# Damorgal/Biprojection-Multimodal-Transformer

Hardware: AMD Instinct MI355X
Metric: training samples/sec (fwd+bwd) BPMulT hidden=768, 3-modal unaligned, at 1/2/4/8 MI355X (higher is better)
Workload: dtype bf16; 1 GPU; BPMulT hidden=768 3-modal unaligned: IEMOCAP-shape synthetic mmtrvat d=768 H=12 layers=8 L/V/A=20/500/400->512; per_gpu_batch=8, global_batch=8, parallelism=dp1, world=1, dropout=README rates (attn .1/0/0, relu .1, res .1, embed .25)

## Files before the change

biprojection-multimodal-transformer_amd/_lib.py:

```python
from __future__ import annotations

import ctypes as C
import os
import subprocess

import torch

_HERE = os.path.dirname(os.path.abspath(__file__))
CSRC = os.path.join(_HERE, "csrc")
LIB_PATH = os.environ.get("BPMULT_LIB", os.path.join(_HERE, "libbpmult_hip.so"))
SOURCES = ("gemm.hip", "attention.hip", "attn_maps.hip", "attn_dbias.hip", "rows_pack.hip", "rows_norm.hip", "rows_elem.hip", "adam.hip", "bert_embed.hip", "loss.hip", "eval.hip", "tail.hip", "frontend.hip", "prof.hip")
HEADERS = ("bpm_common.h", "bpm_launch.h", "bpm_prof.h", "gemm_dma.h", "rows_common.h", "attn_common.h")
ARCH = "gfx950"
PROF_KINDS = {"gemm_nt": 0, "gemm_nn": 1, "gemm_tn": 2, "attn_fwd": 3, "attn_bwd_dq": 4, "attn_bwd_dkv": 5,
              "gemm_dma_nt": 13, "gemm_dma_nn": 14, "gemm_dma_tn": 15, "attn_maps": 16, "attn_bwd_dbias": 17}

ABI_VERSION = 5
LAB_LIB_PATH = os.path.join(_HERE, "..", "build", "lab", "libbpmult_hip_lab.so")
BPM_F32, BPM_BF16, BPM_BF16X3 = 0, 1, 2
GEMM_NT, GEMM_NN, GEMM_TN = 0, 1, 2
OUT_F32, OUT_CT, OUT_HEADS = 0, 1, 2
F_ACCUM, F_RELU, F_ATOMIC, F_KPAD, F_BACKGROUND = 1, 2, 4, 8, 16
F_A_OVERLAP, F_B_OVERLAP = 32, 64
F_CT_NARROW, F_BATCHED = 128, 256
# ... 26 lines not shown
    if not force and fresh():
        return out
    os.makedirs(objdir, exist_ok=True)
    os.makedirs(os.path.dirname(os.path.abspath(out)), exist_ok=True)
    hipcc = os.environ.get("HIPCC", "/opt/rocm/bin/hipcc")
    common = [hipcc, f"--offload-arch={ARCH}", "-O3", "-std=c++17", "-fPIC"] + list(flags)

    def compile_one(src):
        obj = os.path.join(objdir, os.path.basename(src)[:-4] + ".o")
        if not force and os.path.exists(obj) and os.path.getmtime(obj) >= max(os.path.getmtime(src), newest_hdr):
            return obj
        tmp = f"{obj}.{os.getpid()}.tmp"
        cmd = common + ["-c", src, "-o", tmp]
        if verbose:
            print(" ".join(cmd))
        subprocess.run(cmd, check=True)
        os.replace(tmp, obj)
        return obj

    with open(os.path.join(objdir, ".lock"), "w") as lock:
        fcntl.flock(lock, fcntl.LOCK_EX)
        try:
            if not force and fresh():
                return out
            with ThreadPoolExecutor(max_workers=min(4, os.cpu_count() or 1)) as ex:
                objs = list(ex.map(compile_one, srcs))
            tmp = f"{out}.{os.getpid()}.tmp"
            cmd = [hipcc, f"--offload-arch={ARCH}", "-shared", "-fPIC", "-o", tmp] + objs
            if verbose:
                print(" ".join(cmd))
            subprocess.run(cmd, check=True)
            os.replace(tmp, out)
        finally:
            fcntl.flock(lock, fcntl.LOCK_UN)
    return out


def build_lab(force: bool = False) -> str:
    return build(force=force, out=LAB_LIB_PATH, flags=("-DBPM_LAB",))


class GemmProblem(C.Structure):
    _fields_ = [("A", C.c_void_p), ("B", C.c_void_p), ("C", C.c_void_p),
                ("M", C.c_int), ("N", C.c_int), ("K", C.c_int),
                ("lda", C.c_int), ("ldb", C.c_int), ("ldc", C.c_int),
                ("bias_n", C.c_void_p), ("bias_m", C.c_void_p),
                ("resid", C.c_void_p), ("ldr", C.c_int),
                ("gate", C.c_void_p), ("ldg", C.c_int), ("gate_scale", C.c_float),
                ("alpha", C.c_float), ("drop_p", C.c_float), ("drop_site", C.c_uint32),
                ("colsum", C.c_void_p),
                ("flags", C.c_int), ("out_kind", C.c_int), ("splitk", C.c_int),
                ("heads_B", C.c_int), ("heads_H", C.c_int), ("heads_T", C.c_int),
                ("heads_dh", C.c_int), ("heads_dhp", C.c_int), ("colsum_a", C.c_void_p),
                ("batch", C.c_int), ("batch_stride_a", C.c_int), ("batch_stride_b", C.c_int), ("batch_stride_c", C.c_int)]


class AttnProblem(C.Structure):
    _fields_ = [("Q", C.c_void_p), ("K", C.c_void_p), ("V", C.c_void_p),
                ("O", C.c_void_p), ("ldo", C.c_int), ("lse", C.c_void_p),
                ("dO", C.c_void_p), ("delta", C.c_void_p),
                ("dQ", C.c_void_p), ("lddq", C.c_int),
                ("dK", C.c_void_p), ("lddk", C.c_int),
                ("dV", C.c_void_p), ("lddv", C.c_int),
                ("B", C.c_int), ("H", C.c_int), ("T", C.c_int), ("S", C.c_int),
                ("dh", C.c_int), ("dhp", C.c_int), ("mask_off", C.c_int),
                ("dq_scale", C.c_float), ("drop_p", C.c_float), ("drop_site", C.c_uint32),
                ("q_pos0", C.c_int), ("q_stride", C.c_int),
                ("dS", C.c_void_p), ("Pd", C.c_void_p), ("xs_b", C.c_int), ("xs_h", C.c_int), ("xs_q", C.c_int)]


class AttnKMask(C.Structure):
    _fields_ = [("mask", C.c_void_p), ("ldm", C.c_int)]


class AttnAMask(C.Structure):
    _fields_ = [("mask", C.c_void_p), ("ldm", C.c_int), ("maskT", C.c_void_p), ("ldt", C.c_int)]


class AttnHMask(C.Structure):
    _fields_ = [("mask", C.c_void_p), ("ldm", C.c_int), ("maskT", C.c_void_p), ("ldt", C.c_int),
                ("head_stride", C.c_int64), ("head_strideT", C.c_int64)]


class AttnDBias(C.Structure):
    _fields_ = [("dB", C.c_void_p), ("lddb", C.c_int), ("head_stride", C.c_int64)]


class GeluProblem(C.Structure):
    _fields_ = [("u", C.c_void_p), ("ldu", C.c_int), ("u_is_ct", C.c_int), ("g", C.c_void_p), ("ldg", C.c_int),
                ("dg", C.c_void_p), ("lddg", C.c_int), ("du", C.c_void_p), ("lddu", C.c_int), ("R", C.c_int), ("C", C.c_int)]


class BertEmbedProblem(C.Structure):
    _fields_ = [("ids", C.c_void_p), ("seg", C.c_void_p), ("word", C.c_void_p), ("pos", C.c_void_p), ("type", C.c_void_p),
                ("V", C.c_int), ("P", C.c_int), ("Tt", C.c_int), ("gamma", C.c_void_p), ("beta", C.c_void_p),
                ("B", C.c_int), ("L", C.c_int), ("x", C.c_void_p), ("xc", C.c_void_p), ("ldc", C.c_int),
                ("s", C.c_void_p), ("mean", C.c_void_p), ("rstd", C.c_void_p), ("bad", C.c_void_p),
                ("drop_p", C.c_float), ("drop_site", C.c_uint32)]


class BertScatterProblem(C.Structure):
    _fields_ = [("ds", C.c_void_p), ("sorted_ids", C.c_void_p), ("perm", C.c_void_p), ("seg", C.c_void_p),
                ("dword", C.c_void_p), ("dpos", C.c_void_p), ("dtype", C.c_void_p),
                ("V", C.c_int), ("Tt", C.c_int), ("B", C.c_int), ("L", C.c_int), ("padding_idx", C.c_int64),
                ("ws", C.c_void_p), ("ws_bytes", C.c_size_t)]


# ... 34 lines not shown
    _fields_ = [("off4", C.c_size_t), ("n4", C.c_uint), ("blk0", C.c_uint), ("dst", C.c_void_p),
                ("rows", C.c_int), ("cols", C.c_int), ("dst_ld", C.c_int), ("group", C.c_int)]


class AdamGroup(C.Structure):
    _fields_ = [("lr", C.c_float), ("beta1", C.c_float), ("beta2", C.c_float), ("eps", C.c_float), ("weight_decay", C.c_float),
                ("decoupled", C.c_int), ("step", C.c_int), ("pad_", C.c_int)]


class AdamSet(C.Structure):
    _fields_ = [("param", C.c_void_p), ("grad", C.c_void_p), ("exp_avg", C.c_void_p), ("exp_avg_sq", C.c_void_p), ("n", C.c_size_t)]


def adam_set_group(set_index: int, group: int) -> int:
    w = (set_index << ADAM_SET_SHIFT) | (group & 0xff)
    return w - (1 << 32) if w >= 1 << 31 else w


class SumsqSeg(C.Structure):
    _fields_ = [("p", C.c_void_p), ("n", C.c_size_t), ("blk0", C.c_uint), ("pad_", C.c_uint)]


class LossDesc(C.Structure):
    _fields_ = [("kind", C.c_int), ("reduction", C.c_int), ("B", C.c_int), ("C", C.c_int),
                ("logits", C.c_void_p), ("ld", C.c_int), ("target", C.c_void_p), ("ldt", C.c_int), ("weight", C.c_void_p),
                ("ignore_index", C.c_int64), ("loss", C.c_void_p), ("dlogits_unit", C.c_void_p), ("ldd", C.c_int),
                ("bad", C.c_void_p), ("ws", C.c_void_p), ("ws_bytes", C.c_size_t)]


class EvalDesc(C.Structure):
    _fields_ = [("kind", C.c_int), ("C", C.c_int), ("capacity", C.c_int), ("max_batches", C.c_int),
                ("score", C.c_void_p), ("predict", C.c_void_p), ("raw", C.c_void_p), ("target", C.c_void_p),
                ("pred", C.c_void_p), ("label", C.c_void_p), ("losses", C.c_void_p), ("bad", C.c_void_p),
                ("logits", C.c_void_p), ("ld", C.c_int), ("targets", C.c_void_p), ("ldt", C.c_int), ("loss", C.c_void_p),
                ("B", C.c_int), ("n0", C.c_int), ("batch_index", C.c_int),
                ("N", C.c_int), ("nbatches", C.c_int), ("result", C.c_void_p), ("counts", C.c_void_p),
                ("ws", C.c_void_p), ("ws_bytes", C.c_size_t)]


class SplitProblem(C.Structure):
    _fields_ = [("src", C.c_void_p), ("dst", C.c_void_p), ("R", C.c_int), ("C", C.c_int), ("ld", C.c_int), ("ldp", C.c_int)]


class EmbedProblem(C.Structure):
    _fields_ = [("x", C.c_void_p), ("out", C.c_void_p), ("T", C.c_int), ("B", C.c_int), ("accumulate", C.c_int),
                ("drop_p", C.c_float), ("drop_site", C.c_uint32), ("pos0", C.c_int), ("pos_stride", C.c_int)]


class KvSourceProblem(C.Structure):
    _fields_ = [("xk", C.c_void_p), ("xv", C.c_void_p), ("T", C.c_int), ("B", C.c_int), ("pos0", C.c_int), ("pos_stride", C.c_int),
                ("drop_p_k", C.c_float), ("drop_site_k", C.c_uint32), ("drop_p_v", C.c_float), ("drop_site_v", C.c_uint32),
                ("khat", C.c_void_p), ("vhat", C.c_void_p), ("ld", C.c_int),
                ("mean_k", C.c_void_p), ("rstd_k", C.c_void_p), ("mean_v", C.c_void_p), ("rstd_v", C.c_void_p),
                ("gk", C.c_void_p), ("gv", C.c_void_p), ("dxk", C.c_void_p), ("dxv", C.c_void_p)]


class LnProblem(C.Structure):
    _fields_ = [("x", C.c_void_p), ("gamma", C.c_void_p), ("beta", C.c_void_p),
                ("out", C.c_void_p), ("ldo", C.c_int), ("out_f32", C.c_int),
                ("mean", C.c_void_p), ("rstd", C.c_void_p), ("R", C.c_int),
                ("dy", C.c_void_p), ("ldy", C.c_int), ("add", C.c_void_p), ("dx", C.c_void_p),
                ("dgamma", C.c_void_p), ("dbeta", C.c_void_p),
                ("cast", C.c_void_p), ("ldc", C.c_int), ("cast_colsum", C.c_void_p),
                ("drop_p", C.c_float), ("drop_site", C.c_uint32)]


class CastProblem(C.Structure):
    _fields_ = [("a", C.c_void_p), ("lda", C.c_int), ("a_is_ct", C.c_int),
                ("b", C.c_void_p), ("ldb", C.c_int),
                ("dst_ct", C.c_void_p), ("ldd", C.c_int), ("ct_cols", C.c_int),
                ("dst_f32", C.c_void_p), ("ldf", C.c_int),
                ("colsum", C.c_void_p), ("R", C.c_int), ("C", C.c_int),
                ("drop_p", C.c_float), ("drop_site", C.c_uint32)]


class GmuProblem(C.Structure):
    _fields_ = [("a1", C.c_void_p), ("a2", C.c_void_p), ("ag", C.c_void_p), ("x1", C.c_void_p), ("x2", C.c_void_p),
                ("out", C.c_void_p), ("dout", C.c_void_p), ("da1", C.c_void_p), ("da2", C.c_void_p), ("dag", C.c_void_p),
                ("ldg", C.c_int), ("dx1", C.c_void_p), ("dx2", C.c_void_p), ("R", C.c_int)]


class AddnProblem(C.Structure):
    _fields_ = [("out", C.c_void_p), ("src", C.c_void_p * 8), ("n_in", C.c_int), ("count", C.c_size_t)]


class ExpandProblem(C.Structure):
    _fields_ = [("q", C.c_void_p), ("dO", C.c_void_p), ("qexp", C.c_void_p), ("dOexp", C.c_void_p), ("Pd", C.c_void_p),
                ("dbias", C.c_void_p), ("B", C.c_int), ("H", C.c_int), ("T", C.c_int), ("S", C.c_int), ("dh", C.c_int),
                ("dhp", C.c_int), ("ld", C.c_int)]


class TailDesc(C.Structure):
    _fields_ = [("B", C.c_int), ("d", C.c_int), ("n", C.c_int), ("C", C.c_int), ("N", C.c_int * 3),
                ("top", C.c_void_p * 3), ("mid", C.c_void_p * 3), ("extra", C.c_void_p),
                ("Wh", C.c_void_p * 4), ("Wg", C.c_void_p * 4),
                ("W1", C.c_void_p), ("b1", C.c_void_p), ("W2", C.c_void_p), ("b2", C.c_void_p), ("Wo", C.c_void_p), ("bo", C.c_void_p),
                ("out_dropout", C.c_float), ("drop_site", C.c_uint32),
                ("x", C.c_void_p), ("z", C.c_void_p), ("t", C.c_void_p), ("h", C.c_void_p), ("p1", C.c_void_p), ("y", C.c_void_p),
                ("logits", C.c_void_p)]


class TailGrads(C.Structure):
    _fields_ = [("dlogits", C.c_void_p), ("dz", C.c_void_p), ("dWh", C.c_void_p * 4), ("dWg", C.c_void_p * 4),
                ("dW1", C.c_void_p), ("db1", C.c_void_p), ("dW2", C.c_void_p), ("db2", C.c_void_p), ("dWo", C.c_void_p), ("dbo", C.c_void_p),
                ("dtop", C.c_void_p * 3), ("dmid", C.c_void_p * 3), ("dextra", C.c_void_p),
                ("dy", C.c_void_p), ("dp1", C.c_void_p), ("dh", C.c_void_p), ("dzp", C.c_void_p), ("dtp", C.c_void_p), ("dx", C.c_void_p)]

# ... 64 lines not shown
    "bpm_grad_sumsq_blocks": [_P, C.c_size_t],
    "bpm_grad_sumsq_ws_bytes": [C.c_uint],
    "bpm_grad_sumsq": [_P, _I, C.c_uint, _F, _F, _P, _P, C.c_size_t, _P, _P],
    "bpm_loss_ws_bytes": [_I, _I, _I, _I],
    "bpm_loss_fwd": [C.POINTER(LossDesc), _P],
    "bpm_loss_bwd": [C.POINTER(LossDesc), _P, _I, _P, _I, _P],
    "bpm_eval_ws_bytes": [_I, _I, _I],
    "bpm_eval_update": [C.POINTER(EvalDesc), _P],
    "bpm_eval_finalize": [C.POINTER(EvalDesc), _P],
    "bpm_eval_image_bytes": [_I, _I, _I, _I],
    "bpm_eval_pack": [C.POINTER(EvalDesc), _I, _I, _I, _I, _P, C.c_size_t, _P],
    "bpm_eval_merge": [C.POINTER(EvalDesc), _P, C.c_size_t, _I, C.POINTER(_I), C.POINTER(_I), _P],
    "bpm_stream_create": [_I, C.POINTER(C.c_void_p)],
    "bpm_stream_priority_range": [C.POINTER(_I), C.POINTER(_I)],
    "bpm_prof_enable": [C.c_uint],
    "bpm_prof_collect": [_I, C.POINTER(C.c_double), C.POINTER(C.c_double), C.POINTER(_I)],
    "bpm_prof_collect2": [_I, C.POINTER(C.c_double), C.POINTER(C.c_double), C.POINTER(C.c_double), C.POINTER(_I)],
}

_lib = None


class HipLibraryError(RuntimeError):
    pass


def load(path: str) -> C.CDLL:
    if not os.path.exists(path):
        raise HipLibraryError(
            f"{path} not found: run `python -c 'import __graft_entry__ as g; g.build()'` "
            "(hipcc --offload-arch=gfx950). The BPMulT hot path has no CPU/PyTorch fallback.")
    L = C.CDLL(path)
    for name, args in SIGNATURES.items():
        fn = getattr(L, name)
        fn.argtypes = args
        fn.restype = C.c_char_p if name == "bpm_error_string" else C.c_size_t if name.endswith("_bytes") else C.c_int
    v = L.bpm_version()
    if v != ABI_VERSION:
        raise HipLibraryError(f"{path}: ABI version {v}, this package binds version {ABI_VERSION} (include/bpmult_hip.h): rebuild it")
    return L


def lib() -> C.CDLL:
    global _lib
    if _lib is None:
        _lib = load(LIB_PATH)
    return _lib


def bind_lab(L: C.CDLL) -> C.CDLL:
    L.bpm_debug_gemm_force.argtypes = [C.c_int]
    L.bpm_debug_attn_pair.argtypes = [C.c_int]
    L.bpm_debug_gemm_choice.argtypes = [C.c_int, C.c_int, C.POINTER(GemmProblem), C.c_int, C.c_int, C.POINTER(C.c_int)]
    L.bpm_debug_rows_dry.argtypes = [C.c_int]
    L.bpm_debug_rows_last.argtypes = [C.c_int, C.c_char_p, C.c_int, C.POINTER(C.c_uint), C.POINTER(C.c_uint), C.POINTER(C.c_void_p)]
    return L


class lab_library:

    def __enter__(self) -> C.CDLL:
        global _lib
        self._prev = _lib
        _lib = bind_lab(load(LAB_LIB_PATH))
        return _lib

    def __exit__(self, *exc) -> None:
        global _lib
        try:
            _lib.bpm_debug_gemm_force(-1)
            _lib.bpm_debug_attn_pair(7)
        finally:
            _lib = self._prev


_prof_mask = 0


def prof_enable(mask: int) -> None:
    global _prof_mask
    lib().bpm_prof_enable(mask)
    _prof_mask = mask


def prof_enabled() -> bool:
    return _prof_mask != 0


_DEBUG_SYNC = bool(int(os.environ.get("BPMULT_DEBUG_SYNC", "0")))


def check(rc: int, what: str) -> None:
    if rc != 0:
        msg = lib().bpm_error_string(rc)
        raise RuntimeError(f"{what} failed (code {rc}): {msg.decode() if msg else '?'}")
    if _DEBUG_SYNC:
        import sys
        import torch
        print(f"[bpmult] {what} ...", end="", file=sys.stderr, flush=True)
        torch.cuda.synchronize()
        print(" ok", file=sys.stderr, flush=True)
```

biprojection-multimodal-transformer_amd/csrc/gemm.hip:

```cpp
#include <cstdlib>
#include <type_traits>

#include "bpm_common.h"
#include "bpm_prof.h"
#include "../../include/bpmult_hip.h"

namespace {

constexpr int BM = 128, BN = 64, WM = 2, WN = 2;
constexpr int NTHREADS = 64 * WM * WN;
constexpr int TM = BM / WM / 16;
constexpr int TN = BN / WN / 16;
constexpr int BPM_TILED_MINW = 5;
constexpr int BPM_SETPRIO = 0;
constexpr int BPM_DEEP_TN = 2;
constexpr int BPM_DEEP_FWD = 1;
constexpr int KS_FWD = 1, KS_WGRAD = 2;
struct Prob {
    const char* X; const char* Y; char* C;
    int M, N, K;
    int ldx, ldy, ldc;
    const float* bias_n; const float* bias_m;
    const float* resid; const char* gate;
    int ldr, ldg; float gate_scale;
    float alpha;
    float* colsum;
    float* colsum_x;
    DropCfg drop;
    int flags;
    int out_kind;
    int hB, hH, hT, hdh, hdhp;
    int tile0, tiles_m, tiles_n, splitk;
};
static_assert(sizeof(Prob) == 168, "Prob layout");

struct Group {
    const uint64_t* seedp;
    int nprob;
    int total_tiles;
    Prob p[BPM_GEMM_MAX_GROUP];
};
static_assert(sizeof(Group) + 16 <= 4096, "the problem table travels as a kernel argument (4 KB)");

BPM_DEV int swz4(int row) { return (-(row >> 2)) & 3; }

template <typename CT>
BPM_DEV void store_ct4(char* C, size_t off_elems, const float (&v)[4], int nvalid) {
    CT* p = (CT*)C + off_elems;
    if (nvalid == 4 && ((off_elems & 3) == 0)) {
        if constexpr (sizeof(CT) == 4) {
            *(f32x4*)p = f32x4{v[0], v[1], v[2], v[3]};
        } else {
            bf16x4 o;
#pragma unroll
            for (int r = 0; r < 4; ++r) o[r] = (bf16_t)v[r];
            *(bf16x4*)p = o;
        }
    } else {
#pragma unroll
        for (int r = 0; r < 4; ++r)
            if (r < nvalid) p[r] = Tr<CT>::from_f(v[r]);
    }
}

template <typename CT>
BPM_DEV void epilogue_tile(const Prob& P, const DropCfg& drop, bool lead, int m, int nb, const f32x4& acc, float (&csum)[4]) {
    if (m >= P.M) return;
    const bool atomic = (P.flags & BPM_GEMM_ATOMIC) != 0;
    const bool accum = (P.flags & BPM_GEMM_ACCUM) != 0;
    const bool relu = (P.flags & BPM_GEMM_RELU) != 0;
    const bool full = nb + 3 < P.N;
    float v[4];
    float bn[4] = {0.f, 0.f, 0.f, 0.f}, rs[4] = {0.f, 0.f, 0.f, 0.f}, gt[4] = {1.f, 1.f, 1.f, 1.f};
    if (lead && P.bias_n) {
        const float* bp = P.bias_n + nb;
        if (full && (((uintptr_t)bp & 15) == 0)) { const f32x4 t = *(const f32x4*)bp; bn[0] = t[0]; bn[1] = t[1]; bn[2] = t[2]; bn[3] = t[3]; }
        else {
#pragma unroll
            for (int q = 0; q < 4; ++q) if (nb + q < P.N) bn[q] = bp[q];
        }
    }
    if (lead && P.resid) {
        const float* rp = P.resid + (size_t)m * P.ldr + nb;
        if (full && (((uintptr_t)rp & 15) == 0)) { const f32x4 t = *(const f32x4*)rp; rs[0] = t[0]; rs[1] = t[1]; rs[2] = t[2]; rs[3] = t[3]; }
// ... 305 lines not shown
        if (KCONTIG) {
            if (SWZ) {
                const int r = lane & 15, g = lane >> 4;
                return *(const typename Tr<CT>::frag*)(img + (r0 + r) * 64 + ((g ^ swz4(r0 + r)) << 4));
            }
            return read_rowfrag<CT>(img, ROW_STRIDE, r0, ks, lane);
        }
        return Tr<CT>::read_tr(img, STRIDE, ks * Tr<CT>::KSTEP, r0, lane, Tr<CT>::TR_CTILE);
    }
};

BPM_DEV const Prob& pick_problem(const Group& grp, int& bid) {
    int pi = 0;
#pragma unroll 1
    for (int i = 1; i < grp.nprob; ++i)
        if (bid >= grp.p[i].tile0) pi = i;
    bid -= grp.p[pi].tile0;
    return grp.p[pi];
}

#ifdef BPM_GEMM_TRACE
__device__ unsigned long long g_trace[8192 * 16];
#define BPM_TRACE(slot) do { if (threadIdx.x == 0 && blockIdx.x < 8192 && (slot) < 16) \
        g_trace[blockIdx.x * 16 + (slot)] = __builtin_amdgcn_s_memrealtime(); } while (0)
#else
#define BPM_TRACE(slot) do { } while (0)
#endif

template <typename CT, bool XK, bool YK, int KSTEPS, bool DEEP = false, bool FAST = false, int BMT = BM>
__global__ __launch_bounds__(NTHREADS) __attribute__((amdgpu_waves_per_eu((!XK && !YK) ? (BMT == 64 ? 6 : 4) : BPM_TILED_MINW, (!XK && !YK) ? (BMT == 64 ? 6 : 4) : BPM_TILED_MINW))) void gemm_tiled_kernel(const Group grp) {
    typedef Side<CT, XK, BMT, KSTEPS, XK && !YK> SX;
    constexpr int TMT = BMT / WM / 16;
    typedef Side<CT, YK, BN, KSTEPS, false> SY;
    constexpr int STAGE = SX::IMG_BYTES + SY::IMG_BYTES;
    __shared__ __attribute__((aligned(16))) char smem[2 * STAGE];

    const int tid = threadIdx.x, lane = tid & 63, wave = tid >> 6;
    const int wm = wave / WN, wn = wave % WN;

    BPM_TRACE(0);
    int bid = xcd_remap(blockIdx.x, gridDim.x);
    const Prob& P = pick_problem(grp, bid);
    if (BPM_BASE_PRIO && XK && !(P.flags & BPM_GEMM_BACKGROUND)) __builtin_amdgcn_s_setprio(BPM_BASE_PRIO);
    const int tiles = P.tiles_m * P.tiles_n;
    const int split = bid / tiles;
    const int t = bid % tiles;
    const int m0 = (t / P.tiles_n) * BMT, n0 = (t % P.tiles_n) * BN;
    const bool batched = (P.flags & BPM_GEMM_BATCHED) != 0;

    constexpr int BK = SX::BK;
    const int nkt_all = (P.K + BK - 1) / BK;
    const int per = batched ? nkt_all : (nkt_all + P.splitk - 1) / P.splitk;
    const int kt_lo = batched ? 0 : split * per;
    const int kt_hi = min(nkt_all, kt_lo + per);

    f32x4 acc[TN][TMT];
#pragma unroll
    for (int a = 0; a < TN; ++a)
#pragma unroll
        for (int b = 0; b < TMT; ++b) acc[a][b] = f32x4{0.f, 0.f, 0.f, 0.f};

    constexpr int XBT = (TMT + WN - 1) / WN;
    [[maybe_unused]] f32x4 xs[XBT];
    [[maybe_unused]] bool do_xs = false;
    if constexpr (!XK && !YK) {
        do_xs = P.colsum_x != nullptr && n0 == 0;
#pragma unroll
        for (int b = 0; b < XBT; ++b) xs[b] = f32x4{0.f, 0.f, 0.f, 0.f};
    }
    auto compute = [&](const char* ix) {
        const char* iy = ix + SX::IMG_BYTES;
#pragma unroll
        for (int ks = 0; ks < KSTEPS; ++ks) {
            typename Tr<CT>::frag fx[TMT], fy[TN];
#pragma unroll
            for (int b = 0; b < TMT; ++b) fx[b] = SX::frag(ix, wm * (BMT / WM) + 16 * b, ks, lane);
            if constexpr (!XK && !YK) {
                if (do_xs) {
                    typename Tr<CT>::frag one;
#pragma unroll
                    for (int j = 0; j < Tr<CT>::EPC; ++j) one[j] = Tr<CT>::from_f(1.0f);
#pragma unroll
                    for (int b = 0; b < TMT; ++b)
                        if (b / XBT == wn) xs[b % XBT] = Tr<CT>::mma(one, fx[b], xs[b % XBT]);
                }
            }
#pragma unroll
            for (int a = 0; a < TN; ++a) fy[a] = SY::frag(iy, wn * (BN / WN) + 16 * a, ks, lane);
            if (BPM_SETPRIO) __builtin_amdgcn_s_setprio(1);
#pragma unroll
            for (int a = 0; a < TN; ++a)
#pragma unroll
                for (int b = 0; b < TMT; ++b) acc[a][b] = Tr<CT>::mma(fy[a], fx[b], acc[a][b]);
            if (BPM_SETPRIO) __builtin_amdgcn_s_setprio(0);
        }
    };

    const char* const Xp = P.X + (batched ? (size_t)split * (size_t)P.hB * sizeof(CT) : (size_t)0);
    const char* const Yp = P.Y + (batched ? (size_t)split * (size_t)P.hH * sizeof(CT) : (size_t)0);
    const int ldx = P.ldx, ldy = P.ldy, Mb = P.M, Nb = P.N, Kb = P.K;
    [[maybe_unused]] __amdgpu_buffer_rsrc_t rsx, rsy;
    [[maybe_unused]] int vx[SX::PER_THREAD], vy[SY::PER_THREAD];
    [[maybe_unused]] int stepx = 0, stepy = 0;
    if constexpr (FAST) {
        constexpr int E = Tr<CT>::EPC;
        const int kceil = (Kb + BK - 1) / BK * BK;
        const int wx = XK ? kceil : (Mb + E - 1) / E * E, wy = YK ? kceil : (Nb + E - 1) / E * E;
        rsx = __builtin_amdgcn_make_buffer_rsrc((void*)Xp, 0, ((XK ? Mb : Kb) - 1) * ldx * (int)sizeof(CT) + ((P.flags & BPM_GEMM_A_OVERLAP) ? wx : min(wx, ldx)) * (int)sizeof(CT), 0x00020000);
        rsy = __builtin_amdgcn_make_buffer_rsrc((void*)Yp, 0, ((YK ? Nb : Kb) - 1) * ldy * (int)sizeof(CT) + ((P.flags & BPM_GEMM_B_OVERLAP) ? wy : min(wy, ldy)) * (int)sizeof(CT), 0x00020000);
        SX::voffsets(ldx, m0, tid, vx);
        SY::voffsets(ldy, n0, tid, vy);
        stepx = SX::stage_step(ldx);
        stepy = SY::stage_step(ldy);
    }
    auto LD = [&](int kt, u32x4 (&rx_)[SX::PER_THREAD], u32x4 (&ry_)[SY::PER_THREAD], uint32_t& mx_, uint32_t& my_) {
        if constexpr (FAST) {
            SX::load_fast(rsx, vx, kt * stepx, rx_);
            SY::load_fast(rsy, vy, kt * stepy, ry_);
            mx_ = 0xFFFFFFFFu; my_ = 0xFFFFFFFFu;
        } else {
            mx_ = SX::load(Xp, ldx, m0, Mb, kt * BK, Kb, rx_, tid);
            my_ = SY::load(Yp, ldy, n0, Nb, kt * BK, Kb, ry_, tid);
        }
    };
    if constexpr (DEEP) {
        u32x4 rx0[SX::PER_THREAD], ry0[SY::PER_THREAD], rx1[SX::PER_THREAD], ry1[SY::PER_THREAD];
        uint32_t mx0 = 0, my0 = 0, mx1 = 0, my1 = 0;
        auto ld0 = [&](int kt) { LD(kt, rx0, ry0, mx0, my0); };
        auto ld1 = [&](int kt) { LD(kt, rx1, ry1, mx1, my1); };
        auto st0 = [&](char* img) { SX::store(img, rx0, mx0, tid); SY::store(img + SX::IMG_BYTES, ry0, my0, tid); };
        auto st1 = [&](char* img) { SX::store(img, rx1, mx1, tid); SY::store(img + SX::IMG_BYTES, ry1, my1, tid); };
        ld0(kt_lo);
        st0(smem);
        ld1(kt_lo + 1);
        __syncthreads();
        BPM_TRACE(1);
        int cur = 0;
#pragma unroll 1
        for (int kt = kt_lo; kt < kt_hi; kt += 2) {
            ld0(kt + 2);
            compute(smem + cur * STAGE);
            if (kt + 1 < kt_hi) st1(smem + (cur ^ 1) * STAGE);
            __syncthreads();
            BPM_TRACE(2 + kt - kt_lo);
            cur ^= 1;
            if (kt + 1 >= kt_hi) break;
            ld1(kt + 3);
            compute(smem + cur * STAGE);
            if (kt + 2 < kt_hi) st0(smem + (cur ^ 1) * STAGE);
            __syncthreads();
            BPM_TRACE(3 + kt - kt_lo);
            cur ^= 1;
        }
    } else {
        u32x4 rx[SX::PER_THREAD], ry[SY::PER_THREAD];
        uint32_t mx = 0, my = 0;
        LD(kt_lo, rx, ry, mx, my);
        SX::store(smem, rx, mx, tid);
        SY::store(smem + SX::IMG_BYTES, ry, my, tid);
        __syncthreads();
        BPM_TRACE(1);
        int cur = 0;
#pragma unroll 1
        for (int kt = kt_lo; kt < kt_hi; ++kt) {
            const bool more = kt + 1 < kt_hi;
            LD(kt + 1, rx, ry, mx, my);
            compute(smem + cur * STAGE);
            if (more) {
                char* nx = smem + (cur ^ 1) * STAGE;
                SX::store(nx, rx, mx, tid);
                SY::store(nx + SX::IMG_BYTES, ry, my, tid);
            }
            __syncthreads();
            BPM_TRACE(2 + kt - kt_lo);
            cur ^= 1;
        }
    }

// ... 164 lines not shown
    int force_dma;
    int two_mask;
    bool narrow_dma;
};
#ifdef BPM_LAB
int env_int(const char* name, int unset) { const char* v = std::getenv(name); return v ? std::atoi(v) : unset; }
Lab g_lab = {-1, env_int("BPMULT_TWO_MASK", 7), env_int("BPMULT_NARROW_DMA", 1) != 0};
#else
constexpr Lab g_lab = {-1, 7, true};
#endif

int num_cus() {
    static int ncu = 0;
    if (!ncu) {
        int dev = 0;
        hipDeviceProp_t prop;
        ncu = (hipGetDevice(&dev) == hipSuccess && hipGetDeviceProperties(&prop, dev) == hipSuccess && prop.multiProcessorCount > 0)
                  ? prop.multiProcessorCount : 256;
    }
    return ncu;
}

bool bounded_ok(const bpm_gemm_problem& q, int variant, int sz) {
    const bool xk = variant != BPM_GEMM_TN, yk = variant == BPM_GEMM_NT;
    const int stage_b = 64 * (variant == BPM_GEMM_NT ? KS_FWD : 1);
    const bool aov = (q.flags & BPM_GEMM_A_OVERLAP) != 0, bov = (q.flags & BPM_GEMM_B_OVERLAP) != 0;
    bool ok = (q.flags & BPM_GEMM_KPAD_ZERO) != 0;
    if (xk) ok = ok && (aov ? q.K % 64 == 0 : ((long)q.lda * sz) % stage_b == 0 && (long)q.K <= q.lda);
    if (yk) ok = ok && (bov ? q.K % 64 == 0 : ((long)q.ldb * sz) % stage_b == 0 && (long)q.K <= q.ldb);
    const long bx = ((long)(xk ? q.M : q.K) - 1) * q.lda * sz + (long)(aov ? (xk ? q.K : q.M) : q.lda) * sz;
    const long by = ((long)(yk ? q.N : q.K) - 1) * q.ldb * sz + (long)(bov ? (yk ? q.K : q.N) : q.ldb) * sz;
    return ok && bx < (1l << 31) - 65536 && by < (1l << 31) - 65536;
}

int check_group(int dtype, int variant, const bpm_gemm_problem* probs, int nprob) {
    if (nprob < 1 || nprob > BPM_GEMM_MAX_GROUP || !probs) return BPM_ERR_ARG;
    if (variant != BPM_GEMM_NT && variant != BPM_GEMM_NN && variant != BPM_GEMM_TN) return BPM_ERR_ARG;
    if (dtype != BPM_F32 && dtype != BPM_BF16 && dtype != BPM_BF16X3) return BPM_ERR_ARG;
    const int sz = dtype == BPM_F32 ? 4 : 2;
    bool fast = true, overlap = false;
    for (int i = 0; i < nprob && fast; ++i) {
        overlap = overlap || (probs[i].flags & (BPM_GEMM_A_OVERLAP | BPM_GEMM_B_OVERLAP)) != 0;
        fast = bounded_ok(probs[i], variant, sz);
    }
    if (overlap && !fast) return BPM_ERR_ARG;
    for (int i = 0; i < nprob; ++i) {
        const bpm_gemm_problem& q = probs[i];
        if (q.M < 1 || q.N < 1 || q.K < 1 || !q.A || !q.B || !q.C) return BPM_ERR_ARG;
        if ((q.lda * sz) % 16 || (q.ldb * sz) % 16) return BPM_ERR_ALIGN;
        if (((uintptr_t)q.A | (uintptr_t)q.B) & 15) return BPM_ERR_ALIGN;
        if (q.colsum_a && (variant != BPM_GEMM_TN || q.splitk > 1)) return BPM_ERR_ARG;
        if (q.out_kind == BPM_OUT_HEADS && (q.heads_B < 1 || q.heads_dh < 1 || q.heads_H * q.heads_dh != q.N)) return BPM_ERR_ARG;
        if (q.splitk > 1 && !((q.flags & BPM_GEMM_ATOMIC) && q.out_kind == BPM_OUT_F32)) return BPM_ERR_ARG;
        if (q.flags & BPM_GEMM_BATCHED) {
            const uintptr_t al = (uintptr_t)q.C | (uintptr_t)q.bias_n;
            if (dtype == BPM_BF16X3 || q.batch < 1 || q.batch > 4096 || q.splitk > 1 || q.out_kind == BPM_OUT_HEADS || q.bias_m || q.resid ||
                q.gate || q.colsum || q.colsum_a || q.drop_p != 0.f || (q.flags & (BPM_GEMM_ATOMIC | BPM_GEMM_ACCUM)) ||
                (q.N & 3) || (q.ldc & 3) || (al & 15) || q.batch_stride_a < 0 || q.batch_stride_b < 0 || q.batch_stride_c < 0 ||
                ((q.batch_stride_a * sz) & 15) || ((q.batch_stride_b * sz) & 15) || (q.batch_stride_c & 3))
                return BPM_ERR_ARG;
        }
    }
    return 0;
}

struct GroupShape {
    bool fast = true;
    bool legal = true;
    bool big = true;
    bool narrow = true;
    bool skinny = true;
    bool xs_any = false;
    long kmin = 1l << 30, kmax = 0, nmax = 0, mmax = 0;
    long t128 = 0;
    long wg128 = 0;
    long t256 = 0, t320 = 0, tiles_narrow = 0;
};

GroupShape summarise(int dtype, int variant, const bpm_gemm_problem* probs, int nprob) {
    const bool x3 = dtype == BPM_BF16X3, xk = variant != BPM_GEMM_TN, yk = variant == BPM_GEMM_NT;
    const int sz = dtype == BPM_F32 ? 4 : 2;
    GroupShape s;
    for (int i = 0; i < nprob; ++i) {
        const bpm_gemm_problem& q = probs[i];
        s.fast = s.fast && bounded_ok(q, variant, sz);
        const long kceil = ((long)q.K + DK - 1) / DK * DK;
        bool legal = q.splitk <= 1 && !(q.flags & (BPM_GEMM_ATOMIC | BPM_GEMM_BATCHED)) && (!xk || (q.flags & BPM_GEMM_A_OVERLAP) || kceil <= q.lda) &&
                     (!yk || (q.flags & BPM_GEMM_B_OVERLAP) || kceil <= q.ldb);
        if (x3) {
            const long pa = q.lda / 2, pb = q.ldb / 2, m128 = ((long)q.M + 127) / 128 * 128, n128 = ((long)q.N + 127) / 128 * 128;
            legal = legal && !(q.flags & (BPM_GEMM_A_OVERLAP | BPM_GEMM_B_OVERLAP)) && (q.lda & 1) == 0 && (q.ldb & 1) == 0 &&
                    (xk ? kceil <= pa : m128 <= pa) && (yk ? kceil <= pb : n128 <= pb) && (pa * 2) % 16 == 0 && (pb * 2) % 16 == 0;
        }
        const uintptr_t al = (uintptr_t)q.bias_n | (uintptr_t)q.resid | (uintptr_t)q.C | (uintptr_t)q.gate;
        s.legal = s.legal && legal && (q.N & 3) == 0 && (al & 15) == 0 && ((q.ldr | q.ldc | q.ldg) & 3) == 0 && !q.bias_m &&
                  !(q.resid && (q.flags & BPM_GEMM_ACCUM));
        const long tm = (q.M + 255) / 256, tn = (q.N + 255) / 256, tn_narrow = (q.N + 127) / 128;
        s.big = s.big && q.M >= 256 && q.N >= 256 && q.K >= 256 && (double)q.M * q.N >= 0.8 * (double)(tm * 256) * (double)(tn * 256);
        s.narrow = s.narrow && q.M >= 256 && q.N >= 128 && q.K >= 256 && (double)q.M * q.N >= 0.75 * (double)(tm * 256) * (double)(tn_narrow * 128);
        s.skinny = s.skinny && q.M <= 16 && q.splitk <= 1 &&
                   !(q.flags & (BPM_GEMM_ATOMIC | BPM_GEMM_A_OVERLAP | BPM_GEMM_B_OVERLAP | BPM_GEMM_BATCHED)) &&
                   ((long)q.lda * sz) % 64 == 0 && (variant != BPM_GEMM_NT || ((long)q.ldb * sz) % 64 == 0);
        s.xs_any = s.xs_any || q.colsum_a != nullptr;
        s.kmin = q.K < s.kmin ? q.K : s.kmin;
        s.kmax = q.K > s.kmax ? q.K : s.kmax;
        s.nmax = q.N > s.nmax ? q.N : s.nmax;
        s.mmax = q.M > s.mmax ? q.M : s.mmax;
        const long t = (long)((q.M + BM - 1) / BM) * ((q.N + BN - 1) / BN);
        s.t128 += t * (q.splitk > 1 ? q.splitk : 1);
        s.wg128 += t * ((q.flags & BPM_GEMM_BATCHED) ? q.batch : q.splitk > 1 ? q.splitk : 1);
        s.t256 += tm * tn;
        s.t320 += (q.M + 319) / 320 * tn;
        s.tiles_narrow += tm * tn_narrow;
    }
    return s;
}

Choice choose(const GroupShape& s, int dtype, int variant, int nprob, int ncu, const Lab& lab) {
    const bool x3 = dtype == BPM_BF16X3, tn = variant == BPM_GEMM_TN;
    int dma = -1;
    if ((dtype == BPM_BF16 || x3) && s.fast && s.legal && (lab.force_dma != -2 || x3)) {
        const bool big = x3 || (s.big && !(tn && s.t256 * 8 < (long)ncu * 5));
        if (lab.force_dma >= 0 && !x3) dma = lab.force_dma == K_DMA_TALL && tn ? -1 : lab.force_dma;
        else if (big) {
            dma = tn ? K_DMA_2 : K_DMA_3;
            if (!tn) {
                const long r256 = (s.t256 + ncu - 1) / ncu, r320 = (s.t320 + ncu - 1) / ncu;
                if (r320 * 320 * 21 < r256 * 256 * 20) dma = K_DMA_TALL;
            }
            const bool nt = variant == BPM_GEMM_NT;
            const bool two_tn = (lab.two_mask & 1) && tn && !s.xs_any && s.kmin >= 1024 && s.mmax <= 1024;
            const bool kv = (lab.two_mask & 2) && nt && nprob >= 12 && s.nmax <= 1024;
            const bool fc1 = (lab.two_mask & 4) && nt && s.nmax >= 2048 && s.kmax <= 1024;
            if (!x3 && (two_tn || kv || fc1)) dma = K_DMA_TWO;
        }
        else if (lab.narrow_dma && !tn && s.narrow && s.tiles_narrow >= ncu) dma = K_DMA_TWO;
    }
    if (dma >= 0) return {x3 ? (dma == K_DMA_2 ? K_X3_2 : dma == K_DMA_3 ? K_X3_3 : K_X3_TALL) : (Kernel)dma, DMA_CFGS[dma].bm, DMA_CFGS[dma].bn};
    if (x3) return {K_NONE, 0, 0};
    if (!tn && s.fast && s.skinny) return {K_SKINNY, 16, 64};
    if (!tn) return {s.fast ? K_TILED_FAST : K_TILED_BOUNDED, BM, BN};
    if (s.fast) return s.t128 < 2 * 256 ? Choice{K_TN_64, 64, BN} : Choice{K_TILED_FAST, BM, BN};
    return {s.wg128 >= 2 * 256 ? K_TN_SHORT : K_TN_LONG, BM, BN};
}

int check_choice(const Choice& c, const bpm_gemm_problem* probs, int nprob) {
    if (c.kernel == K_NONE) return BPM_ERR_ARG;
    for (int i = 0; i < nprob; ++i) {
        const bpm_gemm_problem& q = probs[i];
        const int ntiles = (q.N + c.bn - 1) / c.bn;
        if (q.out_kind == BPM_OUT_CT && !(q.flags & BPM_GEMM_CT_NARROW) && ntiles * c.bn < q.ldc) return BPM_ERR_ARG;
        if ((q.flags & BPM_GEMM_BATCHED) && (is_dma(c.kernel) || c.kernel == K_SKINNY)) return BPM_ERR_ARG;
    }
    return 0;
}

void fill_group(const Choice& c, const bpm_gemm_problem* probs, int nprob, uint64_t seed, Group& g) {
    g.seedp = bpm_seed_ptr(seed);
    g.nprob = nprob;
    int tile = 0;
    for (int i = 0; i < nprob; ++i) {
        const bpm_gemm_problem& q = probs[i];
        Prob& p = g.p[i];
        p.X = (const char*)q.A; p.Y = (const char*)q.B; p.C = (char*)q.C;
        p.M = q.M; p.N = q.N; p.K = q.K;
        p.ldx = q.lda; p.ldy = q.ldb; p.ldc = q.ldc;
        p.bias_n = q.bias_n; p.bias_m = q.bias_m;
        p.resid = q.resid; p.ldr = q.ldr;
        p.gate = (const char*)q.gate; p.ldg = q.ldg; p.gate_scale = q.gate_scale;
        p.alpha = q.alpha;
        p.drop = bpm_make_drop(q.drop_p, seed, q.drop_site);
        p.colsum = q.colsum;
        p.colsum_x = q.colsum_a;
        p.flags = q.flags; p.out_kind = q.out_kind;
        p.hB = q.heads_B; p.hH = q.heads_H; p.hT = q.heads_T; p.hdh = q.heads_dh; p.hdhp = q.heads_dhp;
        p.tile0 = tile;
        p.tiles_m = (q.M + c.bm - 1) / c.bm;
        p.tiles_n = (q.N + c.bn - 1) / c.bn;
        p.splitk = q.splitk > 1 ? q.splitk : 1;
        if (q.flags & BPM_GEMM_BATCHED) {
            p.splitk = q.batch;
            p.hB = q.batch_stride_a; p.hH = q.batch_stride_b; p.hT = q.batch_stride_c;
        }
        tile += p.tiles_m * p.tiles_n * p.splitk;
    }
    g.total_tiles = tile;
}

int plan_group(int dtype, int variant, const bpm_gemm_problem* probs, int nprob, uint64_t seed, int ncu, GroupShape& shape, Choice& c, Group& g) {
    if (const int err = check_group(dtype, variant, probs, nprob)) return err;
    shape = summarise(dtype, variant, probs, nprob);
    c = choose(shape, dtype, variant, nprob, ncu ? ncu : num_cus(), g_lab);
    if (const int err = check_choice(c, probs, nprob)) return err;
    fill_group(c, probs, nprob, seed, g);
    return 0;
}

void work_estimate(int dtype, const bpm_gemm_problem* probs, int nprob, double& flops, double& bytes) {
    const int sz = dtype == BPM_F32 ? 4 : 2;
    flops = bytes = 0;
    for (int i = 0; i < nprob; ++i) {
        const bpm_gemm_problem& q = probs[i];
        flops += 2.0 * q.M * (double)q.N * q.K * ((q.flags & BPM_GEMM_BATCHED) ? q.batch : 1);
        const double mn = (double)q.M * q.N;
        bytes += ((double)q.M + q.N) * q.K * sz + mn * (q.out_kind == BPM_OUT_F32 ? 4 : sz);
        if (q.resid) bytes += mn * 4;
        if (q.gate) bytes += mn * sz;
        if (q.out_kind == BPM_OUT_F32 && (q.flags & BPM_GEMM_ACCUM)) bytes += mn * 4;
    }
}

typedef void (*KernelFn)(const Group);

int launch_variant(int variant, KernelFn nt, KernelFn nn, KernelFn tn, int threads, const Group& g, hipStream_t s) {
    const KernelFn kernel = variant == BPM_GEMM_NT ? nt : variant == BPM_GEMM_NN ? nn : tn;
    if (!kernel) return BPM_ERR_ARG;
    hipLaunchKernelGGL(kernel, dim3(g.total_tiles), dim3(threads), 0, s, g);
    BPM_CHECK_LAUNCH();
    return 0;
}

template <int WMD, int WND, int TMW, int NS, bool X3 = false, int DKT = DK>
int launch_dma(int variant, bool xs, const Group& g, hipStream_t s) {
    KernelFn tn = nullptr;
    if constexpr ((16 * TMW * WMD) % 128 == 0)
        tn = xs ? gemm_dma_kernel<false, false, WMD, WND, TMW, NS, true, X3, DKT> : gemm_dma_kernel<false, false, WMD, WND, TMW, NS, false, X3, DKT>;
    return launch_variant(variant, gemm_dma_kernel<true, true, WMD, WND, TMW, NS, false, X3, DKT>,
                          gemm_dma_kernel<true, false, WMD, WND, TMW, NS, false, X3, DKT>, tn, 64 * WMD * WND, g, s);
}

template <typename CT>
int launch(const Choice& c, int variant, bool xs, const Group& g, hipStream_t s) {
    switch (c.kernel) {
        case K_DMA_0: return launch_dma<2, 2, 4, 2>(variant, xs, g, s);
        case K_DMA_1: return launch_dma<4, 2, 4, 2>(variant, xs, g, s);
        case K_DMA_2: return launch_dma<2, 4, 8, 2>(variant, xs, g, s);
        case K_DMA_3: return launch_dma<4, 4, 4, 2>(variant, xs, g, s);
        case K_DMA_4: return launch_dma<2, 2, 4, 3>(variant, xs, g, s);
        case K_DMA_TALL: return launch_dma<2, 4, 10, 2>(variant, xs, g, s);
        case K_DMA_TWO: return launch_dma<4, 2, 4, 3, false, 32>(variant, xs, g, s);
        case K_X3_2: return launch_dma<2, 4, 8, 2, true>(variant, xs, g, s);
        case K_X3_3: return launch_dma<4, 4, 4, 2, true>(variant, xs, g, s);
        case K_X3_TALL: return launch_dma<2, 4, 10, 2, true>(variant, xs, g, s);
        case K_SKINNY: return launch_variant(variant, gemm_skinny_kernel<CT, true>, gemm_skinny_kernel<CT, false>, nullptr, 256, g, s);
        case K_TILED_FAST:
            return launch_variant(variant, gemm_tiled_kernel<CT, true, true, KS_FWD, BPM_DEEP_FWD != 0, true>,
                                  gemm_tiled_kernel<CT, true, false, 1, BPM_DEEP_FWD != 0, true>,
                                  gemm_tiled_kernel<CT, false, false, 1, true, true>, NTHREADS, g, s);
        case K_TILED_BOUNDED:
            return launch_variant(variant, gemm_tiled_kernel<CT, true, true, KS_FWD, BPM_DEEP_FWD != 0>,
                                  gemm_tiled_kernel<CT, true, false, 1, BPM_DEEP_FWD != 0>, nullptr, NTHREADS, g, s);
        case K_TN_64: return launch_variant(variant, nullptr, nullptr, gemm_tiled_kernel<CT, false, false, 1, true, true, 64>, NTHREADS, g, s);
        case K_TN_SHORT: return launch_variant(variant, nullptr, nullptr, gemm_tiled_kernel<CT, false, false, 1, BPM_DEEP_TN != 0>, NTHREADS, g, s);
        case K_TN_LONG:
            return launch_variant(variant, nullptr, nullptr, BPM_DEEP_TN == 2 ? gemm_tiled_kernel<CT, false, false, 1, true>
                                                                              : gemm_tiled_kernel<CT, false, false, KS_WGRAD, false>, NTHREADS, g, s);
        case K_NONE: break;
    }
    return BPM_ERR_ARG;
}

}

#ifdef BPM_LAB
extern "C" int bpm_debug_gemm_force(int cfg) {
    if (cfg < -2 || cfg >= N_DMA_CFGS) return BPM_ERR_ARG;
    g_lab.force_dma = cfg;
    return 0;
}

extern "C" int bpm_debug_gemm_choice(int dtype, int variant, const bpm_gemm_problem* probs, int nprob, int ncu, int* out) {
    GroupShape shape;
    Choice c;
    Group g;
    if (ncu < 1 || !out) return BPM_ERR_ARG;
    if (const int err = plan_group(dtype, variant, probs, nprob, 0, ncu, shape, c, g)) return err;
    out[0] = c.kernel; out[1] = c.bm; out[2] = c.bn; out[3] = g.total_tiles;
    for (int i = 0; i < nprob; ++i) {
        const Prob& p = g.p[i];
        out[4 + 4 * i] = p.tile0; out[5 + 4 * i] = p.tiles_m; out[6 + 4 * i] = p.tiles_n; out[7 + 4 * i] = p.splitk;
    }
    return 0;
}
#endif

#ifdef BPM_GEMM_TRACE
extern "C" int bpm_debug_trace(unsigned long long* out, int nblocks) {
    if (nblocks > 8192) nblocks = 8192;
    return (int)hipMemcpyFromSymbol(out, HIP_SYMBOL(g_trace), sizeof(unsigned long long) * 16 * nblocks);
}
#endif

extern "C" int bpm_gemm_grouped(int dtype, int variant, const bpm_gemm_problem* probs, int nprob, uint64_t seed, void* stream) {
    GroupShape shape;
    Choice c;
    Group g;
    if (const int err = plan_group(dtype, variant, probs, nprob, seed, 0, shape, c, g)) return err;
    double flops, bytes;
    work_estimate(dtype, probs, nprob, flops, bytes);
    hipStream_t s = (hipStream_t)stream;
    BpmProfScope prof((is_dma(c.kernel) ? BPM_K_GEMM_DMA_NT : BPM_K_GEMM_NT) + variant, s, flops, bytes);
    return dtype == BPM_F32 ? launch<float>(c, variant, shape.xs_any, g, s) : launch<bf16_t>(c, variant, shape.xs_any, g, s);
}
```

biprojection-multimodal-transformer_amd/csrc/gemm_dma.h:

```cpp

constexpr int BPM_EPI_AHEAD = 1;
constexpr int BPM_DMA_EARLY = 1;
#ifndef BPM_DMA_ABLATE
#define BPM_DMA_ABLATE 0
#endif
#ifdef BPM_GEMM_TRACE
#define BPM_TRACE_CLK(slot) do { if (threadIdx.x == 0 && blockIdx.x < 8192) { \
        g_trace[blockIdx.x * 16 + (slot)] = __builtin_amdgcn_s_memtime(); \
        g_trace[blockIdx.x * 16 + (slot) + 1] = __builtin_amdgcn_s_memrealtime(); } } while (0)
#else
#define BPM_TRACE_CLK(slot) do { } while (0)
#endif
constexpr int DK = 64;
constexpr int DROW = 128;

BPM_DEV int desc_bytes(int rows, int ld, int width, int sz, bool overlap = false) { return ((rows - 1) * ld + (overlap ? width : min(width, ld))) * sz; }

BPM_DEV int dma_row_off(int row, int c) { return row * DROW + ((c ^ ((row >> 1) & 7)) << 4); }
BPM_DEV int dma_col_off(int krow, int ch) { return krow * 256 + ((ch ^ (((krow & 3) << 2) | ((krow >> 2) & 3))) << 4); }

template <int N> BPM_DEV void dma_wait() {
    static_assert(N >= 0 && N < 64, "vmcnt immediate");
    asm volatile("s_waitcnt vmcnt(%0)" ::"n"(N) : "memory");
}
// ... 140 lines not shown
        const int q = r >> 2, p = r & 3;
        const char* sub = img + (r0 >> 7) * SUB_BYTES;
        const int ch = ((r0 & 127) >> 3) + (p >> 1);
        const int k0 = 32 * ks + 8 * g + q;
        typedef bf16x4 __attribute__((address_space(3))) * lds4;
        const bf16x4 lo = __builtin_amdgcn_ds_read_tr16_b64_v4bf16((lds4)(sub + dma_col_off(k0, ch) + 8 * (p & 1)));
        const bf16x4 hi = __builtin_amdgcn_ds_read_tr16_b64_v4bf16((lds4)(sub + dma_col_off(k0 + 4, ch) + 8 * (p & 1)));
        bf16x8 f;
#pragma unroll
        for (int j = 0; j < 4; ++j) { f[j] = lo[j]; f[4 + j] = hi[j]; }
        return f;
    }
};

template <typename SX, typename SY, int Q, int F = 0>
BPM_DEV void dma_issue_part(__amdgpu_buffer_rsrc_t rsx, __amdgpu_buffer_rsrc_t rsy, char* bx, int vx, int vy, int sx, int sy,
                            int ldx, int ldy, int wave) {
    constexpr int LPS = SX::PER_WAVE + SY::PER_WAVE;
    if constexpr (F < LPS) {
        if constexpr ((F * 4) / LPS == Q) {
            if constexpr (F < SX::PER_WAVE) SX::template issue_one<F>(rsx, bx, vx, sx, ldx, wave);
            else SY::template issue_one<F - SX::PER_WAVE>(rsy, bx + SX::IMG_BYTES, vy, sy, ldy, wave);
        }
        dma_issue_part<SX, SY, Q, F + 1>(rsx, rsy, bx, vx, vy, sx, sy, ldx, ldy, wave);
    }
}

template <bool XK, bool YK, int WMD, int WND, int TMW, int NS, bool XS = false, bool X3 = false, int DKT = DK>
__global__ __launch_bounds__(64 * WMD * WND) __attribute__((amdgpu_waves_per_eu(DKT == 32 ? 4 : (WMD * WND + 3) / 4)))
void gemm_dma_kernel(const Group grp) {
    typedef typename std::conditional<X3, float, bf16_t>::type OT;
    static_assert(!XS || (!XK && !YK), "column sums of X belong to the weight-gradient product");
    constexpr int NW = WMD * WND, BMD = 16 * TMW * WMD, BND = 64 * WND, WROWS = 16 * TMW;
    typedef DmaSide<XK, BMD, NW, DKT> SX;
    typedef DmaSide<YK, BND, NW, DKT> SY;
    constexpr int KSPS = DKT / 32;
    constexpr int STAGE = SX::IMG_BYTES + SY::IMG_BYTES;
    constexpr int LPS = SX::PER_WAVE + SY::PER_WAVE;
    static_assert(NS == 2 || NS == 3, "2 or 3 stages");
    static_assert(DKT == 64 || !X3, "the split-operand products use 64-k stages");
    static_assert(TMW == 4 || TMW == 8 || TMW == 10, "wave tile 64 x 64, 128 x 64 or 160 x 64");
    __shared__ __attribute__((aligned(1024))) char smem[NS * STAGE];

    const int tid = threadIdx.x, lane = tid & 63;
    const int wave = __builtin_amdgcn_readfirstlane(tid >> 6);
    const int wm = wave / WND, wn = wave % WND;

    BPM_TRACE_CLK(0);
    int bid = xcd_remap(blockIdx.x, gridDim.x);
    const Prob& P = pick_problem(grp, bid);
    if (BPM_BASE_PRIO && XK && !(P.flags & BPM_GEMM_BACKGROUND)) __builtin_amdgcn_s_setprio(BPM_BASE_PRIO);
    const int m0 = (bid / P.tiles_n) * BMD, n0 = (bid % P.tiles_n) * BND;
    const int nk1 = (P.K + DKT - 1) / DKT;
    const int nkt = X3 ? 3 * nk1 : nk1;

    const __amdgpu_buffer_rsrc_t rsx = __builtin_amdgcn_make_buffer_rsrc((void*)P.X, 0, X3 ? (XK ? P.M : P.K) * P.ldx * 2 : desc_bytes(XK ? P.M : P.K, P.ldx, XK ? nkt * DKT : (P.M + 7) & ~7, 2, (P.flags & BPM_GEMM_A_OVERLAP) != 0), 0x00020000);
    const __amdgpu_buffer_rsrc_t rsy = __builtin_amdgcn_make_buffer_rsrc((void*)P.Y, 0, X3 ? (YK ? P.N : P.K) * P.ldy * 2 : desc_bytes(YK ? P.N : P.K, P.ldy, YK ? nkt * DKT : (P.N + 7) & ~7, 2, (P.flags & BPM_GEMM_B_OVERLAP) != 0), 0x00020000);
    const int vx = SX::voffset(P.ldx, m0, wave, lane), vy = SY::voffset(P.ldy, n0, wave, lane);
    const int stepx = SX::stage_step(P.ldx), stepy = SY::stage_step(P.ldy);
    const int ldx = P.ldx, ldy = P.ldy;

    auto seg_of = [&](int kt) { return !X3 ? 0 : (kt >= 2 * nk1 ? 2 : (kt >= nk1 ? 1 : 0)); };
    auto part = [&](int kt, int buf, auto Q) {
        const int seg = seg_of(kt), kk = kt - seg * nk1;
        dma_issue_part<SX, SY, decltype(Q)::value>(rsx, rsy, smem + buf * STAGE, vx, vy, kk * stepx + (seg == 2 ? ldx : 0),
                                                   kk * stepy + (seg == 1 ? ldy : 0), ldx, ldy, wave);
    };
    auto stage = [&](int kt, int buf) {
        part(kt, buf, std::integral_constant<int, 0>{}); part(kt, buf, std::integral_constant<int, 1>{});
        part(kt, buf, std::integral_constant<int, 2>{}); part(kt, buf, std::integral_constant<int, 3>{});
    };

    f32x4 acc[4][TMW];
#pragma unroll
    for (int a = 0; a < 4; ++a)
#pragma unroll
        for (int b = 0; b < TMW; ++b) acc[a][b] = f32x4{0.f, 0.f, 0.f, 0.f};
    constexpr int XB = (TMW + WND - 1) / WND;
    [[maybe_unused]] f32x4 xs[XB];
    [[maybe_unused]] bool do_xs = false;
    if constexpr (XS) {
        do_xs = P.colsum_x != nullptr && n0 == 0;
#pragma unroll
        for (int b = 0; b < XB; ++b) xs[b] = f32x4{0.f, 0.f, 0.f, 0.f};
    }

#pragma unroll
    for (int s = 0; s < NS - 1; ++s)
        if (s < nkt) stage(s, s);

    int buf = 0;
#pragma unroll 1
    for (int kt = 0; kt < nkt; ++kt) {
        if (kt == 1) BPM_TRACE_CLK(2);
        if (NS == 3 && kt + 1 < nkt) dma_wait<LPS>();
        else dma_wait<0>();
        asm volatile("s_waitcnt lgkmcnt(0)" ::: "memory");
        __builtin_amdgcn_s_barrier();
        const bool more = kt + NS - 1 < nkt;
        const int nbuf = buf == 0 ? NS - 1 : buf - 1;
        const char* ix = smem + buf * STAGE;
        const char* iy = ix + SX::IMG_BYTES;
        auto step = [&](auto KS) {
            constexpr int ks = decltype(KS)::value;
            constexpr bool YLATE = DKT == 32 && XS;
            bf16x8 fx[TMW], fy[4];
#pragma unroll
            for (int b = 0; b < TMW; ++b) fx[b] = SX::frag(ix, wm * WROWS + 16 * b, ks, lane);
#pragma unroll
            for (int a = 0; a < (YLATE ? 2 : 4); ++a) fy[a] = SY::frag(iy, wn * 64 + 16 * a, ks, lane);
// ... 110 lines not shown
```

biprojection-multimodal-transformer_amd/csrc/rows_norm.hip:

```cpp
#include "rows_common.h"

namespace {
struct EmbP { const float* x; float* out; int T, B; int accumulate; int pos0, pstride; DropCfg drop; };

BPM_DEV bool emb_wide(const EmbP& P, const float* table, int d, size_t total) {
    return (d & 3) == 0 && total < (1ull << 32) && (((uintptr_t)P.x | (uintptr_t)P.out | (uintptr_t)table) & 15) == 0;
}

__global__ void embed_pos_fwd_kernel(const Grp<EmbP> grp, const float* __restrict__ table, int d, float scale) {
    unsigned bid = blockIdx.x, nblk;
    const EmbP& P = pick(grp, bid, nblk);
    const DropCfg drop = bpm_resolve_drop(P.drop, grp.seedp);
    const size_t total = (size_t)P.T * P.B * d;
    if (emb_wide(P, table, d, total)) {
        const uint32_t total4 = (uint32_t)(total >> 2), ud = (uint32_t)d;
        for (uint32_t q = bid * NT + threadIdx.x; q < total4; q += nblk * NT) {
            const uint32_t i = 4u * q, row = i / ud, c = i - row * ud;
            const int t = (int)(row / (uint32_t)P.B);
            const int pos = (P.x[(size_t)row * ud] != 0.f) ? P.pos0 + t * P.pstride + 1 : 0;
            f32x4 v = scale * *(const f32x4*)(P.x + i) + *(const f32x4*)(table + (size_t)pos * ud + c);
            if (drop.thresh != 0) {
                float d0, d1, d2, d3;
                bpm_drop_mult4(drop, i, d0, d1, d2, d3);
                v *= f32x4{d0, d1, d2, d3};
// ... 481 lines not shown
    if (!ln_vec_ok(q, n, d, true, ct_size)) return 0;
    c = LnChoice{true, d, 8, 64, nullptr};
    bool sums = false;
    for (int i = 0; i < n; ++i) {
        if (q[i].cast && q[i].ldc > c.span) c.span = q[i].ldc;
        sums = sums || q[i].dgamma || (q[i].cast && q[i].cast_colsum);
        if (((uintptr_t)q[i].dgamma | (uintptr_t)q[i].dbeta | (uintptr_t)q[i].cast_colsum) & 15) ws = nullptr;
    }
    if (ws && sums) {
        const float* rows[3 * BPM_MAX_GROUP];
        int nr = 0;
        for (int i = 0; i < n; ++i) {
            if (q[i].dgamma) { rows[nr++] = q[i].dgamma; rows[nr++] = q[i].dbeta; }
            if (q[i].cast && q[i].cast_colsum) rows[nr++] = q[i].cast_colsum;
        }
        for (int a = 0; a < nr && ws; ++a)
            for (int b = a + 1; b < nr; ++b)
                if (rows[a] && rows[a] == rows[b]) { ws = nullptr; break; }
    }
    if (ws && sums) {
        size_t blocks = 0;
        for (int i = 0; i < n; ++i) blocks += blocks_for((size_t)q[i].R, c.rows, c.cap);
        if (((uintptr_t)ws & 15) || ws_bytes < (blocks * 3 * d + LN_WS_HEAD) * sizeof(float)) return BPM_ERR_ARG;
        c.ws = (float*)ws;
    }
    return 0;
}

extern "C" int bpm_ln_bwd_ws(int dtype, const bpm_ln_problem* q, int n, int d, uint64_t seed, void* ws, size_t ws_bytes, void* stream) {
    if (dtype != BPM_F32 && dtype != BPM_BF16) return BPM_ERR_ARG;
    Grp<LnP> g;
    if (const int rc = fill_ln(g, q, n, d, true, seed)) return rc;
    LnChoice c;
    if (const int rc = choose_ln_bwd(q, n, d, dtype == BPM_BF16 ? 2 : 4, ws, ws_bytes, c)) return rc;
    ln_blocks(g, c);
    return with_ct(dtype, [&](auto ct) {
        using CT = decltype(ct);
        if (c.vec) return with_width(VecWidths(), c.span, [&](auto w) {
            return launch<ln_bwd_vec_kernel<CT, decltype(w)::value>>(g.blk0[n], NT, stream, g, d, c.ws);
        });
        return with_width(RowWidths(), c.span, [&](auto w) {
            return launch<ln_bwd_kernel<CT, decltype(w)::value>>(g.blk0[n], NT, stream, g, d);
        });
    });
}

extern "C" int bpm_ln_bwd(int dtype, const bpm_ln_problem* q, int n, int d, uint64_t seed, void* stream) {
    return bpm_ln_bwd_ws(dtype, q, n, d, seed, nullptr, 0, stream);
}

namespace {
struct KvP {
    const float* xk; const float* xv; int T, B, pos0, pstride; DropCfg dk, dv;
    void* khat; void* vhat; int ld; float* mk; float* rk; float* mv; float* rv;
    const float* gk; const float* gv; float* dxk; float* dxv;
};

BPM_DEV f32x4 kv_opaque(f32x4 v) {
    asm("" : "+v"(v));
    return v;
}

BPM_DEV float kv_opaque1(float v) {
    asm("" : "+v"(v));
    return v;
}
BPM_DEV f32x4 kv_fma4(f32x4 a, f32x4 b, f32x4 c) {
    return f32x4{__builtin_fmaf(a[0], b[0], c[0]), __builtin_fmaf(a[1], b[1], c[1]), __builtin_fmaf(a[2], b[2], c[2]), __builtin_fmaf(a[3], b[3], c[3])};
}

BPM_DEV f32x4 kv_embed4(f32x4 x, f32x4 tab, float scale, const DropCfg& drop, uint32_t i0, f32x4& mult) {
    f32x4 v = scale * x + tab;
    mult = f32x4{1.f, 1.f, 1.f, 1.f};
    if (drop.thresh != 0) {
        float d0, d1, d2, d3;
        bpm_drop_mult4(drop, i0, d0, d1, d2, d3);
        mult = f32x4{d0, d1, d2, d3};
        v *= mult;
    }
    return kv_opaque(v);
}

template <typename CT, int NV>
BPM_DEV void kv_norm_store(f32x4 (&v)[NV], int lane, int nch, float inv_d, float eps, int row, void* out, int ld, float* mean, float* rstd) {
    float s = 0.f;
#pragma unroll
    for (int e = 0; e < NV; ++e) s += sum4(v[e]);
    const float mu = wave_sum(s) * inv_d;
    float qq = 0.f;
#pragma unroll
    for (int e = 0; e < NV; ++e) {
        const int q = lane + 64 * e;
        f32x4 t = v[e] - mu;
        if (q >= nch) t = f32x4{0.f, 0.f, 0.f, 0.f};
        v[e] = t;
        qq += sum4(t * t);
    }
    const float rs = rsqrtf(wave_sum(qq) * inv_d + eps);
    if (lane == 0) { mean[row] = mu; rstd[row] = rs; }
#pragma unroll
    for (int e = 0; e < NV; ++e) {
        const int q = lane + 64 * e;
        if (q < nch) put4<CT>(out, (size_t)row * ld + 4 * q, v[e] * rs + 0.f);
        else if (4 * q < ld) put4<CT>(out, (size_t)row * ld + 4 * q, f32x4{0.f, 0.f, 0.f, 0.f});
    }
}

template <typename CT, int NV>
__global__ __launch_bounds__(NT) void kv_source_fwd_kernel(const Grp<KvP> grp, const float* __restrict__ table, int d, float scale, float eps) {
    if (BPM_BASE_PRIO) __builtin_amdgcn_s_setprio(BPM_BASE_PRIO);
    unsigned bid = blockIdx.x, nblk;
    const KvP& P = pick(grp, bid, nblk);
    const DropCfg dk = bpm_resolve_drop(P.dk, grp.seedp), dv = bpm_resolve_drop(P.dv, grp.seedp);
    const int lane = threadIdx.x & 63;
    const int wpb = NT / 64;
    const int nch = d >> 2, R = P.T * P.B;
    const bool same = P.xk == P.xv;
    const float inv_d = 1.f / d;
    for (int row = bid * wpb + (threadIdx.x >> 6); row < R; row += nblk * wpb) {
        const int t = row / P.B;
        const uint32_t r0 = (uint32_t)row * (uint32_t)d;
        const float* xkr = P.xk + r0;
        const float* xvr = P.xv + r0;
        const int posk = xkr[0] != 0.f ? P.pos0 + t * P.pstride + 1 : 0;
        const int posv = same ? posk : xvr[0] != 0.f ? P.pos0 + t * P.pstride + 1 : 0;
        const float* tk = table + (size_t)posk * d;
        const float* tv = table + (size_t)posv * d;
        f32x4 ek[NV], ev[NV];
#pragma unroll
        for (int e = 0; e < NV; ++e) {
            const int q = lane + 64 * e;
            const int qc = q < nch ? q : 0;
            const f32x4 xk4 = *(const f32x4*)(xkr + 4 * qc), tk4 = *(const f32x4*)(tk + 4 * qc);
            f32x4 xv4 = xk4, tv4 = tk4, m;
            if (!same) { xv4 = *(const f32x4*)(xvr + 4 * qc); tv4 = *(const f32x4*)(tv + 4 * qc); }
            const f32x4 a = kv_embed4(xk4, tk4, scale, dk, r0 + 4u * (uint32_t)qc, m);
            const f32x4 b = kv_embed4(xv4, tv4, scale, dv, r0 + 4u * (uint32_t)qc, m);
            ek[e] = q < nch ? a : f32x4{0.f, 0.f, 0.f, 0.f};
            ev[e] = q < nch ? b : f32x4{0.f, 0.f, 0.f, 0.f};
        }
        kv_norm_store<CT, NV>(ek, lane, nch, inv_d, eps, row, P.khat, P.ld, P.mk, P.rk);
        kv_norm_store<CT, NV>(ev, lane, nch, inv_d, eps, row, P.vhat, P.ld, P.mv, P.rv);
    }
}

template <int NV, bool SAME>
__global__ __launch_bounds__(NT) void kv_source_bwd_kernel(const Grp<KvP> grp, const float* __restrict__ table, int d, float scale) {
    if (BPM_BASE_PRIO) __builtin_amdgcn_s_setprio(BPM_BASE_PRIO);
    constexpr int U = SAME ? 2 : 1;
    constexpr int NS = SAME ? 1 : 2;
    unsigned bid = blockIdx.x, nblk;
    const KvP& P = pick(grp, bid, nblk);
    const DropCfg dk = bpm_resolve_drop(P.dk, grp.seedp), dv = bpm_resolve_drop(P.dv, grp.seedp);
    const int lane = threadIdx.x & 63, wv = threadIdx.x >> 6;
    const int wpb = NT / 64;
    const int nch = d >> 2, R = P.T * P.B;
    const bool merge = P.dxv == nullptr || P.dxv == P.dxk;
    const float inv_d = 1.f / d;
    for (int row0 = (bid * wpb + wv) * U; row0 < R; row0 += nblk * wpb * U) {
        f32x4 xs[U][NS][NV], tb[U][NS][NV], g[U][2][NV];
        float mu[U][2], rs[U][2];
#pragma unroll
        for (int u = 0; u < U; ++u) {
            const int row = row0 + u;
            const int rc = row < R ? row : row0;
            const int t = rc / P.B;
            const uint32_t r0 = (uint32_t)rc * (uint32_t)d;
            mu[u][0] = P.mk[rc]; rs[u][0] = P.rk[rc];
            mu[u][1] = P.mv[rc]; rs[u][1] = P.rv[rc];
#pragma unroll
            for (int s = 0; s < NS; ++s) {
                const float* xr = (s ? P.xv : P.xk) + r0;
                const int pos = xr[0] != 0.f ? P.pos0 + t * P.pstride + 1 : 0;
                const float* tr = table + (size_t)pos * d;
#pragma unroll
                for (int e = 0; e < NV; ++e) {
                    const int q = lane + 64 * e;
                    const int qc = q < nch ? q : 0;
                    xs[u][s][e] = *(const f32x4*)(xr + 4 * qc);
                    tb[u][s][e] = *(const f32x4*)(tr + 4 * qc);
                }
            }
#pragma unroll
            for (int e = 0; e < NV; ++e) {
                const int q = lane + 64 * e;
                const int qc = q < nch ? q : 0;
                g[u][0][e] = *(const f32x4*)(P.gk + r0 + 4 * qc);
                g[u][1][e] = *(const f32x4*)(P.gv + r0 + 4 * qc);
            }
        }
#pragma unroll
        for (int u = 0; u < U; ++u) {
            const int row = row0 + u;
            const bool rok = row < R;
            const uint32_t r0 = (uint32_t)(rok ? row : row0) * (uint32_t)d;
#pragma unroll
            for (int side = 0; side < 2; ++side) {
                const int s = SAME ? 0 : side;
                const DropCfg& drop = side ? dv : dk;
                f32x4 xh[NV], mult[NV];
                float s1 = 0.f, s2 = 0.f;
#pragma unroll
                for (int e = 0; e < NV; ++e) {
                    const int q = lane + 64 * e;
                    const bool ok = rok && q < nch;
                    const f32x4 emb = kv_embed4(xs[u][s][e], tb[u][s][e], scale, drop, r0 + 4u * (uint32_t)(q < nch ? q : 0), mult[e]);
                    const f32x4 dyv = ok ? g[u][side][e] : f32x4{0.f, 0.f, 0.f, 0.f};
                    xh[e] = ok ? (emb - mu[u][side]) * rs[u][side] : f32x4{0.f, 0.f, 0.f, 0.f};
                    s1 += sum4(dyv);
                    s2 += sum4(dyv * xh[e]);
                    g[u][side][e] = dyv;
                }
                s1 = wave_sum(s1);
                if constexpr (NV != 1) s1 = kv_opaque1(s1 * inv_d);
                s2 = kv_opaque1(wave_sum(s2) * inv_d);
#pragma unroll
                for (int e = 0; e < NV; ++e) {
                    f32x4 t = NV == 1 ? kv_fma4(f32x4{-inv_d, -inv_d, -inv_d, -inv_d}, f32x4{s1, s1, s1, s1}, g[u][side][e]) : g[u][side][e] - s1;
                    t = kv_fma4(-xh[e], f32x4{s2, s2, s2, s2}, kv_opaque(t));
                    const f32x4 rs4 = f32x4{rs[u][side], rs[u][side], rs[u][side], rs[u][side]};
                    const f32x4 dl = kv_opaque(kv_fma4(rs4, t, f32x4{0.f, 0.f, 0.f, 0.f}));
                    f32x4 v = scale * dl;
                    if (drop.thresh != 0) v *= mult[e];
                    g[u][side][e] = kv_opaque(v);
                }
            }
            if (!rok) continue;
#pragma unroll
            for (int e = 0; e < NV; ++e) {
                const int q = lane + 64 * e;
                if (q < nch) {
                    if (merge) {
                        *(f32x4*)(P.dxk + r0 + 4 * q) = g[u][0][e] + g[u][1][e];
                    } else {
                        *(f32x4*)(P.dxk + r0 + 4 * q) = g[u][0][e];
                        *(f32x4*)(P.dxv + r0 + 4 * q) = g[u][1][e];
                    }
                }
            }
        }
    }
}
}

static int fill_kv(Grp<KvP>& g, const bpm_kv_source_problem* q, int n, const float* table, int table_rows, int d, uint64_t seed,
                   bool bwd, int ct_size) {
    if (!grp_begin(g, q, n, seed) || !table || d < 4 || d % 4 || d > 4 * 64 * 4 || ((uintptr_t)table & 15)) return BPM_ERR_ARG;
    for (int i = 0; i < n; ++i) {
        const bpm_kv_source_problem& s = q[i];
        if (!s.xk || !s.xv || s.T < 1 || s.B < 1 || s.pos0 < 0 || s.pos_stride < 0) return BPM_ERR_ARG;
        if (!s.mean_k || !s.rstd_k || !s.mean_v || !s.rstd_v) return BPM_ERR_ARG;
        const int pstride = s.pos_stride > 0 ? s.pos_stride : 1;
        if ((long long)table_rows < (long long)s.pos0 + (long long)(s.T - 1) * pstride + 2) return BPM_ERR_ARG;
        if ((unsigned long long)s.T * (unsigned long long)s.B * (unsigned long long)d >= (1ull << 32)) return BPM_ERR_ARG;
        uintptr_t a = (uintptr_t)s.xk | (uintptr_t)s.xv;
        if (bwd) {
            if (!s.gk || !s.gv || !s.dxk) return BPM_ERR_ARG;
            a |= (uintptr_t)s.gk | (uintptr_t)s.gv | (uintptr_t)s.dxk | (uintptr_t)s.dxv;
        } else {
            if (!s.khat || !s.vhat || s.ld < d || s.ld % 4 || s.ld > 4 * 64 * 4) return BPM_ERR_ARG;
            if (((uintptr_t)s.khat | (uintptr_t)s.vhat) % (4 * ct_size)) return BPM_ERR_ARG;
        }
        if (a & 15) return BPM_ERR_ARG;
        KvP& p = g.p[i];
        p.xk = s.xk; p.xv = s.xv; p.T = s.T; p.B = s.B; p.pos0 = s.pos0; p.pstride = pstride;
        p.dk = bpm_make_drop(s.drop_p_k, seed, s.drop_site_k);
        p.dv = bpm_make_drop(s.drop_p_v, seed, s.drop_site_v);
        p.khat = s.khat; p.vhat = s.vhat; p.ld = s.ld;
        p.mk = s.mean_k; p.rk = s.rstd_k; p.mv = s.mean_v; p.rv = s.rstd_v;
        p.gk = s.gk; p.gv = s.gv; p.dxk = s.dxk; p.dxv = s.dxv;
    }
    return 0;
}

struct KvChoice {
    int span;
    bool same;
    int rows_per_wave;
};

static KvChoice choose_kv(const bpm_kv_source_problem* q, int n, int d, bool bwd) {
    KvChoice c = {d, true, 1};
    for (int i = 0; i < n; ++i) {
        if (!bwd && q[i].ld > c.span) c.span = q[i].ld;
        if (q[i].xk != q[i].xv) c.same = false;
    }
    if (bwd && c.same) c.rows_per_wave = 2;
    return c;
}

static void kv_blocks(Grp<KvP>& g, const KvChoice& c) {
    for (int i = 0; i < g.n; ++i) {
        const size_t waves = ((size_t)g.p[i].T * g.p[i].B + c.rows_per_wave - 1) / c.rows_per_wave;
        g.blk0[i + 1] = g.blk0[i] + blocks_for(waves, 4, 4096);
    }
}

extern "C" int bpm_kv_source_fwd(int dtype, const bpm_kv_source_problem* q, int n, const float* table, int table_rows, int d,
                                 float scale, float eps, uint64_t seed, void* stream) {
    if (dtype != BPM_F32 && dtype != BPM_BF16) return BPM_ERR_ARG;
    Grp<KvP> g;
    if (const int rc = fill_kv(g, q, n, table, table_rows, d, seed, false, dtype == BPM_BF16 ? 2 : 4)) return rc;
    const KvChoice c = choose_kv(q, n, d, false);
    kv_blocks(g, c);
    return with_ct(dtype, [&](auto ct) {
        return with_width(VecWidths(), c.span, [&](auto w) {
            return launch<kv_source_fwd_kernel<decltype(ct), decltype(w)::value>>(g.blk0[n], NT, stream, g, table, d, scale, eps);
        });
    });
}

extern "C" int bpm_kv_source_bwd(const bpm_kv_source_problem* q, int n, const float* table, int table_rows, int d, float scale,
                                 uint64_t seed, void* stream) {
    Grp<KvP> g;
    if (const int rc = fill_kv(g, q, n, table, table_rows, d, seed, true, 4)) return rc;
    const KvChoice c = choose_kv(q, n, d, true);
    kv_blocks(g, c);
    return with_width(VecWidths(), c.span, [&](auto w) {
        constexpr int NV = decltype(w)::value;
        return c.same ? launch<kv_source_bwd_kernel<NV, true>>(g.blk0[n], NT, stream, g, table, d, scale)
                      : launch<kv_source_bwd_kernel<NV, false>>(g.blk0[n], NT, stream, g, table, d, scale);
// ... 3 lines not shown
```

biprojection-multimodal-transformer_amd/engine.py:

```python
from __future__ import annotations

import ctypes as C
import math
import os
from collections import defaultdict
from dataclasses import dataclass
from typing import Dict, List, NamedTuple, Optional, Sequence, Tuple

import torch

from . import ops
from ._lib import (BPM_BF16, AdamSeg, adam_set_group, AddnProblem, ExpandProblem, F_CT_NARROW, F_ACCUM, F_BACKGROUND, F_KPAD, F_RELU, GEMM_NN, GEMM_NT, GEMM_TN, OUT_CT, OUT_HEADS,
                   AttnProblem, CastProblem, FoldDesc, GemmProblem, KvSourceProblem, LnProblem, PackDesc,
                   UnfoldDesc)
from .ops import pad32

S_EMB_Q, S_EMB_K, S_EMB_V, S_ATTN, S_RES1, S_RELU, S_RES2, S_ATTN_SELF, S_RES0 = range(9)
SITE_TEXT = 1 << 20


def site(enc_id: int, layer: int, op: int) -> int:
    return (enc_id << 12) | (layer << 4) | op


# ... 355 lines not shown
    for si, (st, group_of) in enumerate(zip(stores, group_ofs)):
        for sg in st._adam_segments({n: group_of.get(n, -1) for n in st.names}, raw=True):
            sg.group = adam_set_group(si, sg.group)
            segs.append(sg)
    return ops.adam_sets_table(segs)


def adam_step_sets(stores: Sequence[ParamStore], table, sets, groups, grad_scale, zero_grad: bool,
                   scale_dev: Optional[torch.Tensor] = None, norm_dev: Optional[torch.Tensor] = None,
                   steps_dev: Optional[torch.Tensor] = None, skipped_dev: Optional[torch.Tensor] = None) -> None:
    sigs = [st.begin_adam_step() for st in stores]
    ops.adam_step_sets(stores[0].dtype, table, sets, groups, grad_scale, zero_grad, scale_dev, norm_dev, steps_dev, skipped_dev)
    for st, sig in zip(stores, sigs):
        st.end_adam_step(sig)


@dataclass
class EncoderDesc:
    prefix: str
    enc_id: int
    T: int
    S: int
    attn_dropout: float
    q_pos0: int = 0
    q_stride: int = 1
    T_full: Optional[int] = None
    tail_rows: bool = False


@dataclass
class GroupCfg:
    d: int
    H: int
    layers: int
    relu_dropout: float
    res_dropout: float
    embed_dropout: float
    attn_mask: bool
    biprojection: bool
    self_only: bool = False


SIDE, JOIN, MARK, WAIT, SIDE2 = "side", "join", "mark", "wait", "side2"


class AttentionMap(NamedTuple):
    weights: torch.Tensor
    query_steps: Optional[Tuple[int, ...]]
_SIDE = os.environ.get("BPMULT_SIDE", "1") != "0"
_DKV_SIDE_ENV = os.environ.get("BPMULT_DKV_SIDE", "auto")
_side_streams: Dict[Tuple[int, int, bool], "torch.cuda.Stream"] = {}
_SIDE_PRIORITY_ENV = os.environ.get("BPMULT_SIDE_PRIORITY", "auto")
_LOWRANK = os.environ.get("BPMULT_LOWRANK", "1") != "0"


_OPEN_FORKS: Dict[int, "torch.cuda.Stream"] = {}


def open_forks() -> List["torch.cuda.Stream"]:
    return list(_OPEN_FORKS.values())


def _side_stream(device, which: int = 1, low: bool = True) -> "torch.cuda.Stream":
    dev_i = device.index if device.index is not None else torch.cuda.current_device()
    if _SIDE_PRIORITY_ENV in ("low", "normal"):
        low = _SIDE_PRIORITY_ENV == "low"
    key = (dev_i, which, bool(low))
    if key not in _side_streams:
        from . import _lib
        out = C.c_void_p()
        with torch.cuda.device(dev_i):
            _lib.check(_lib.lib().bpm_stream_create(int(bool(low)), C.byref(out)), "bpm_stream_create")
        _side_streams[key] = torch.cuda.ExternalStream(out.value, device=torch.device("cuda", dev_i))
    return _side_streams[key]


_SELF_KEYS = dict(q="qh", k="kh", v="vh", o="ao", lse="lse", mid="xmid", dy="dy", dao="dao", delta="delta")
_BIP_SELF_KEYS = dict(q="qs", k="ks", v="vs", o="aos", lse="lses", mid="xmid0", dy="dy0", dao="dao0", delta="delta0")


class EncoderGroupPlan:

    def __init__(self, store: ParamStore, cfg: GroupCfg, encs: Sequence[EncoderDesc], B: int, x3: "Optional[ops.X3Cache]" = None):
        self.store, self.cfg, self.encs, self.B = store, cfg, list(encs), B
        self.x3 = x3 if x3 is not None or not store.x3 else ops.X3Cache(store.device, weights=store.x3_cache)
        self.dtype = store.dtype
        d, H = cfg.d, cfg.H
        if d % H:
            raise ValueError("embed_dim must be divisible by num_heads")
        self.dh = d // H
        self.dhp = dhp_for(self.dh)
        self._kv = not cfg.self_only
        self._lowrank = (_LOWRANK and self._kv and not cfg.biprojection
                         and all(e.T * H * 4 <= d and e.S % 4 == 0 for e in self.encs) and self.dh <= 256)
        self.ld, self.ld4 = pad32(d), pad32(4 * d)
        self.scale = self.dh ** -0.5
        self._kv_fused = (self._kv and os.environ.get("BPMULT_KV_FUSED", "1") != "0"
                          and all(ops.kv_source_ok(d, e.S, B) for e in self.encs))
        self._kv_dst: List[Optional[torch.Tensor]] = [None] * len(self.encs)
        self._kv_keep = None
        self._lnF = 2 if cfg.biprojection else 1
        dev = store.device
        L = cfg.layers
        nacc = sum(L * 2 * d + 16 for e in self.encs)
        self._acc0 = torch.zeros(nacc, device=dev, dtype=torch.float32)
        self._acc_off = 0
        self.buf: List[dict] = [self._alloc(e) for e in self.encs]
        if cfg.biprojection and any(e.T_full is not None for e in self.encs):
            raise ValueError("a gathered query subset is only exact for crossmodal (non-biprojection) encoders")
        self.table = sinusoid_table(max(max(e.T_full or e.T, e.S) for e in self.encs) + 2, d, dev)
        self._ones, self._zeros = torch.ones(d, device=dev), torch.zeros(d, device=dev)
        self._kvsrc = {}
        if self._kv_fused:
            for training in (True, False):
                p = cfg.embed_dropout if training else 0.0
                self._kvsrc[training] = ops.array(KvSourceProblem, [
                    ops.kv_source_problem(None, None, e.S, B, khat=b["khat"], vhat=b["vhat"], ld=self.ld, stats_k=b["stk"],
                                          stats_v=b["stv"], gk=b["Gk"], gv=b["Gv"], dxk=b["dxk"], dxv=b["dxv"], drop_p=p,
                                          drop_site_k=site(e.enc_id, 0, S_EMB_K), drop_site_v=site(e.enc_id, 0, S_EMB_V))
                    for e, b in zip(self.encs, self.buf)])
        lnK = 1 if cfg.biprojection else 0
        self._unfold = []
        for i in range(L if self._kv else 0):
            ud, blk = [], 0
            for e, b in zip(self.encs, self.buf):
                pn = lambda leaf: self._pn(e, i, leaf)
                u = UnfoldDesc()
                u.dWf, u.dbf = b["dWf"][i].data_ptr(), b["dbf"][i].data_ptr()
                u.W = store.p(pn("self_attn.in_proj_weight")).data_ptr() + 4 * d * d
                u.gamma, u.beta = store.p(pn(f"layer_norms.{lnK}.weight")).data_ptr(), store.p(pn(f"layer_norms.{lnK}.bias")).data_ptr()
                u.dW, u.dbias = store.gptr(pn("self_attn.in_proj_weight"), d * d), store.gptr(pn("self_attn.in_proj_bias"), d)
                u.dgamma, u.dbeta = store.gptr(pn(f"layer_norms.{lnK}.weight")), store.gptr(pn(f"layer_norms.{lnK}.bias"))
                u.rows, u.cols, u.ldw, u.blk0 = 2 * d, d, d, blk
                blk += (2 * d + 15) // 16
                ud.append(u)
            self._unfold.append((ops.device_table(ud), len(ud), blk))
        self._dkv_side = _DKV_SIDE_ENV if _DKV_SIDE_ENV != "auto" else "1"
        if _DKV_SIDE_ENV == "auto" and max(e.T for e in self.encs) * B <= 64:
            self._dkv_side = "0"
        self._side_low = d < 512
        self.store.side_low = self._side_low
        self._fwd = {True: self._build_fwd(True), False: self._build_fwd(False)}
        self._maps_ok = False
        self._bwd = {(t, f): self._build_bwd(t, f) for t in (True, False) for f in (True, False)}
        for steps in (*self._fwd.values(), *self._bwd.values()):
            self._check_steps(steps)

    def _alloc(self, e: EncoderDesc) -> dict:
        c, B, d, H, L, ld, ld4, dhp = self.cfg, self.B, self.cfg.d, self.cfg.H, self.cfg.layers, self.ld, self.ld4, self.dhp
        dev, ct = self.store.device, ops.ct_torch(self.dtype)
        z = lambda *s, dt=torch.float32: torch.zeros(*s, device=dev, dtype=dt)
        if not self._kv and (e.S != e.T or e.tail_rows or e.T_full is not None or e.q_pos0 or e.q_stride != 1):
            raise ValueError(f"encoder {e.prefix}: a self-attention-only encoder attends over its own {e.T} time steps "
                             "(S == T, no gathered rows, no tail_rows)")
        has_self = c.biprojection or not self._kv
        R, Rk = e.T * B, e.S * B
        tailp = bool(e.tail_rows)
        if tailp and (not c.biprojection or e.T < 2 or e.T_full is not None):
            raise ValueError("tail_rows: biprojection encoders with at least two query rows (crossmodal encoders gather their rows)")
        Rl, Tl = [R] * L, [e.T] * L
        if tailp:
            Rl[-1], Tl[-1] = 2 * B, 2
        b = dict(R=R, Rk=Rk, Rl=Rl, Tl=Tl, tailp=tailp)
        b["x"] = [z(R, d) for _ in range(L)] + [z(Rl[-1], d)]
        b["out"] = z(Tl[-1], B, d)
        b["stf"] = (z(Rl[-1]), z(Rl[-1]))
        if self._kv:
            if not self._kv_fused:
                b["ke"], b["ve"] = z(Rk, d), z(Rk, d)
            b["khat"], b["vhat"] = z(Rk, ld, dt=ct), z(Rk, ld, dt=ct)
            b["stk"], b["stv"] = (z(Rk), z(Rk)), (z(Rk), z(Rk))
            b["Gk"], b["Gv"] = z(Rk, d), z(Rk, d)
            if self._lowrank:
# ... 12 lines not shown
        acts = [("xn", lambda i: (R, ld), ct),
                ("qh", lambda i: (B, H, Tl[i], dhp), ct), ("kh", lambda i: (B, H, e.S, dhp), ct),
                ("vh", lambda i: (B, H, e.S, dhp), ct), ("ao", lambda i: (Rl[i], ld), ct),
                ("lse", lambda i: (B, H, Tl[i]), torch.float32),
                ("xmid", lambda i: (Rl[i], d), torch.float32), ("xn2", lambda i: (Rl[i], ld), ct),
                ("h1", lambda i: (Rl[i], ld4), ct),
                ("st0m", lambda i: (R,), torch.float32), ("st0r", lambda i: (R,), torch.float32),
                ("st1m", lambda i: (Rl[i],), torch.float32), ("st1r", lambda i: (Rl[i],), torch.float32)]
        if self._kv and c.biprojection:
            acts += [("qs", lambda i: (B, H, Tl[i], dhp), ct), ("ks", lambda i: (B, H, e.T, dhp), ct),
                     ("vs", lambda i: (B, H, e.T, dhp), ct), ("aos", lambda i: (Rl[i], ld), ct),
                     ("lses", lambda i: (B, H, Tl[i]), torch.float32), ("xmid0", lambda i: (Rl[i], d), torch.float32),
                     ("xq", lambda i: (Rl[i], ld), ct), ("st2m", lambda i: (Rl[i],), torch.float32),
                     ("st2r", lambda i: (Rl[i],), torch.float32)]
        for nm, shape, dt in acts:
            b[nm] = [z(*shape(i), dt=dt) for i in range(L)]
        if tailp:
            b["xg"], b["xng"] = z(2 * B, d), z(2 * B, ld, dt=ct)
            b["dxg"], b["dxng"], b["dxs"] = z(2 * B, d), z(2 * B, d), z(R, d)
        b["dx"], b["dxn"] = z(R, d), z(R, d)
        two = lambda *shape: [z(*shape, dt=ct), z(*shape, dt=ct)]
        b["dy"], b["dh1"] = two(R, ld), two(R, ld4)
        b["dyf"] = [z(R, ld, dt=ct) for _ in range(3)]
        if self._kv:
            b["dq"] = two(R, ld)
        if self._kv and c.biprojection:
            b["dy0"] = two(R, ld)
        if has_self:
            b["dqkvs"] = two(R + 1, 3 * ld)
            b["dqs"], b["dks"], b["dvs"] = ([t[:R, w * ld:(w + 1) * ld] for t in b["dqkvs"]] for w in range(3))
        if self._kv:
            b["dao"] = [z(B, H, e.T, dhp, dt=ct) for _ in range(2)]
            b["delta"] = [z(B, H, e.T) for _ in range(2)]
        if has_self:
            k = _BIP_SELF_KEYS if self._kv else _SELF_KEYS
            b[k["dao"]], b[k["delta"]] = z(B, H, e.T, dhp, dt=ct), z(B, H, e.T)
        if self._kv:
            if not self._kv_fused:
                b["dke"], b["dve"] = z(Rk, d), z(Rk, d)
            b["dxk"], b["dxv"] = z(e.S, B, d), z(e.S, B, d)
        b["dxq"] = z(e.T, B, d)
        return b

    def _mask_off(self, T: int, S: int) -> int:
        return 1 + abs(S - T) if self.cfg.attn_mask else 0

    def _pn(self, e: EncoderDesc, i: int, leaf: str) -> str:
        return f"{e.prefix}layers.{i}.{leaf}"

    def _gemm(self, variant, probs, background=False, presplit=()):
        for p in probs:
            p.flags |= F_KPAD | (F_BACKGROUND if background else 0)
        arr = ops.array(GemmProblem, probs)
        arr.x3 = self.x3
        arr.x3_presplit = frozenset(t.data_ptr() for t in presplit)
        return (ops.gemm_grouped, self.dtype, variant, arr)

    def _tail(self, b: dict, i: int) -> bool:
        return b["tailp"] and i == self.cfg.layers - 1

    def _proj(self, e, i, Ain, rows, which, Cout, Tlen):
        d, ld = self.cfg.d, self.ld
        return ops.gemm_problem(Ain, self.store.sptr(self._pn(e, i, "self_attn.in_proj_weight"), which * d * ld), Cout, rows, d, d,
                                ld, ld, 0, bias_n=self.store.p(self._pn(e, i, "self_attn.in_proj_bias"))[which * d:(which + 1) * d],
                                alpha=self.scale if which == 0 else 1.0, out_kind=OUT_HEADS,
                                heads=(self.B, self.cfg.H, Tlen, self.dh, self.dhp))

    def _ln0_fwd(self, t, e, b, i):
        P = lambda leaf: self.store.p(self._pn(e, i, leaf))
        t["ln0"].append(ops.ln_problem(b["x"][i], P("layer_norms.0.weight"), P("layer_norms.0.bias"), b["st0m"][i], b["st0r"][i],
                                       b["R"], out=b["xn"][i], ldo=self.ld))

    def _ln0_bwd(self, t, e, b, i, pr):
        st, c, d = self.store, self.cfg, self.cfg.d
        nxt = {} if i == 0 else dict(cast=b["dyf"][(i - 1) % 3], ldc=self.ld, cast_colsum=st.gptr(self._pn(e, i - 1, "fc2.bias")),
                                     drop_p=pr(c.res_dropout), drop_site=site(e.enc_id, i - 1, S_RES2))
        t["ln0"].append(ops.ln_problem(b["x"][i], st.p(self._pn(e, i, "layer_norms.0.weight")), None, b["st0m"][i], b["st0r"][i],
                                       b["R"], dy=b["dxn"], ldy=d, add=b["dxs"] if self._tail(b, i) else b["dx"], dx=b["dx"],
                                       dgamma=st.gptr(self._pn(e, i, "layer_norms.0.weight")),
                                       dbeta=st.gptr(self._pn(e, i, "layer_norms.0.bias")), **nxt))

    def _self_attn_fwd(self, t, e, b, i, pr, k, res_site):
        st, c, B, d, H, ld = self.store, self.cfg, self.B, self.cfg.d, self.cfg.H, self.ld
        R, Rq, Tq = b["R"], b["Rl"][i], b["Tl"][i]
        x_in, xn = b["x"][i], b["xn"][i]
        xq_in, res_in = xn, x_in
        tail = self._tail(b, i)
        if tail:
            for j, r0 in ((0, 0), (1, R - B)):
                t["s.gather"].append(ops.cast_problem(x_in[r0:r0 + B], d, B, d, dst_f32=b["xg"][j * B:(j + 1) * B], ldf=d))
                t["s.gather"].append(ops.cast_problem(xn[r0:r0 + B], ld, B, d, a_is_ct=True, dst_ct=b["xng"][j * B:(j + 1) * B],
                                                      ldd=ld))
            xq_in, res_in = b["xng"], b["xg"]
        q, kk, v, o, lse = (b[k[n]][i] for n in ("q", "k", "v", "o", "lse"))
        t["s.qkv"] += [self._proj(e, i, xq_in, Rq, 0, q, Tq), self._proj(e, i, xn, R, 1, kk, e.T), self._proj(e, i, xn, R, 2, v, e.T)]
        t["s.att"].append(ops.attn_problem(q, kk, v, o, ld, lse, B, H, Tq, e.T, self.dh, self.dhp, self._mask_off(e.T, e.T),
                                           drop_p=pr(e.attn_dropout), drop_site=site(e.enc_id, i, S_ATTN_SELF),
                                           **(dict(q_pos0=0, q_stride=e.T - 1) if tail else {})))
        t["s.out"].append(ops.gemm_problem(o, st.sptr(self._pn(e, i, "self_attn.out_proj.weight")), b[k["mid"]][i], Rq, d, d, ld, ld,
                                           d, bias_n=st.p(self._pn(e, i, "self_attn.out_proj.bias")), resid=res_in, ldr=d,
                                           drop_p=pr(c.res_dropout), drop_site=site(e.enc_id, i, res_site)))

    def _self_attn_bwd(self, t, e, b, i, pr, k, first, acc1, cast=None):
        st, c, B, d, H, ld = self.store, self.cfg, self.B, self.cfg.d, self.cfg.H, self.ld
        R, Rq, Tq = b["R"], b["Rl"][i], b["Tl"][i]
        GP = lambda leaf, off=0: st.gptr(self._pn(e, i, leaf), off)
        ipw, wo = self._pn(e, i, "self_attn.in_proj_weight"), self._pn(e, i, "self_attn.out_proj.weight")
        par = i & 1
        dy, dqs, dks, dvs = b[k["dy"]][par], b["dqs"][par], b["dks"][par], b["dvs"][par]
        q, kk, v, o, lse, dao, delta = (b[k[n]] for n in ("q", "k", "v", "o", "lse", "dao", "delta"))
        q, kk, v, o, lse = q[i], kk[i], v[i], o[i], lse[i]
        tail = self._tail(b, i)
        xn = b["xn"][i]
        xq_in = b["xng"] if tail else xn
        if cast is not None:
            t["s.cast"].append(ops.cast_problem(cast[0], d, Rq, d, dst_ct=dy, ldd=ld, colsum=GP("self_attn.out_proj.bias"),
                                                drop_p=pr(c.res_dropout), drop_site=site(e.enc_id, i, cast[1])))
        t["s.acts"] += [o, xq_in, xn]
        t["s.wg"].append(ops.gemm_problem(dy, o, GP("self_attn.out_proj.weight"), d, d, Rq, ld, ld, d, flags=first))
        t["s.dgout"].append(ops.gemm_problem(dy, st.sptr(wo), dao, Rq, d, d, ld, ld, 0, out_kind=OUT_HEADS,
                                             heads=(B, H, Tq, self.dh, self.dhp)))
        t["s.att"].append(ops.attn_problem(q, kk, v, o, ld, lse, B, H, Tq, e.T, self.dh, self.dhp, self._mask_off(e.T, e.T),
                                           dO=dao, delta=delta, dQ=dqs, lddq=3 * ld, dK=dks, lddk=3 * ld, dV=dvs, lddv=3 * ld,
                                           dq_scale=self.scale, drop_p=pr(e.attn_dropout), drop_site=site(e.enc_id, i, S_ATTN_SELF),
                                           **(dict(q_pos0=0, q_stride=e.T - 1) if tail else {})))
        for w, src, xin, rows in ((0, dqs, xq_in, Rq), (1, dks, xn, R), (2, dvs, xn, R)):
            t["s.wg"].append(ops.gemm_problem(src, xin, st.gptr(ipw, w * d * d), d, d, rows, 3 * ld, ld, d,
                                              flags=first if w == 0 else acc1,
                                              colsum_a=GP("self_attn.in_proj_bias", w * d)))
        if tail:
            if ld == d:
                t["s.dg_a"].append(ops.gemm_problem(b["dqkvs"][par][:R, ld:], st.sptr(ipw, d * ld), b["dxn"], R, d, 2 * d,
                                                    3 * ld, ld, d))
            else:
                t["s.dg_a"].append(ops.gemm_problem(dks, st.sptr(ipw, d * ld), b["dxn"], R, d, d, 3 * ld, ld, d))
                t["s.dg_b"].append(ops.gemm_problem(dvs, st.sptr(ipw, 2 * d * ld), b["dxn"], R, d, d, 3 * ld, ld, d, flags=F_ACCUM))
            t["s.dgq"].append(ops.gemm_problem(dqs, st.sptr(ipw, 0), b["dxng"], Rq, d, d, 3 * ld, ld, d))
            for j, r0 in ((0, 0), (1, R - B)):
                blk = slice(j * B, (j + 1) * B)
                t["s.scatter"].append(ops.addn_problem(b["dxn"][r0:r0 + B], [b["dxn"][r0:r0 + B], b["dxng"][blk]]))
                t["s.scatter"].append(ops.addn_problem(b["dxs"][r0:r0 + B], [b["dxg"][blk]]))
        elif ld == d:
            t["s.dg_a"].append(ops.gemm_problem(b["dqkvs"][par], st.sptr(ipw, 0), b["dxn"], R, d, 3 * d, 3 * ld, ld, d))
        else:
            t["s.dg_a"].append(ops.gemm_problem(dqs, st.sptr(ipw, 0), b["dxn"], R, d, d, 3 * ld, ld, d))
            t["s.dg_b"].append(ops.gemm_problem(dks, st.sptr(ipw, d * ld), b["dxn"], R, d, d, 3 * ld, ld, d, flags=F_ACCUM))
            t["s.dg_c"].append(ops.gemm_problem(dvs, st.sptr(ipw, 2 * d * ld), b["dxn"], R, d, d, 3 * ld, ld, d, flags=F_ACCUM))

    def _cross_attn_fwd(self, t, e, b, i, pr, q_src, resid):
        st, c, B, d, H, ld = self.store, self.cfg, self.B, self.cfg.d, self.cfg.H, self.ld
        Rq, Tq = b["Rl"][i], b["Tl"][i]
        qpos = dict(q_pos0=0, q_stride=e.T - 1) if self._tail(b, i) else dict(q_pos0=e.q_pos0, q_stride=e.q_stride)
        kvf = self._pn(e, i, KVF)
        t["c.q"].append(self._proj(e, i, q_src, Rq, 0, b["qh"][i], Tq))
        for w, hat, dst in ((0, b["khat"], b["kh"][i]), (1, b["vhat"], b["vh"][i])):
            t["c.kv"].append(ops.gemm_problem(hat, st.sptr(kvf + (".v" if w else ".k")), dst, b["Rk"], d, d, ld, ld, 0,
                                              bias_n=st.fold(kvf, w * d, d), out_kind=OUT_HEADS, heads=(B, H, e.S, self.dh, self.dhp)))
        t["c.att"].append(ops.attn_problem(b["qh"][i], b["kh"][i], b["vh"][i], b["ao"][i], ld, b["lse"][i], B, H, Tq, e.S, self.dh,
                                           self.dhp, self._mask_off(e.T_full or e.T, e.S), drop_p=pr(e.attn_dropout),
                                           drop_site=site(e.enc_id, i, S_ATTN), **qpos))
        t["c.out"].append(ops.gemm_problem(b["ao"][i], st.sptr(self._pn(e, i, "self_attn.out_proj.weight")), b["xmid"][i], Rq, d, d,
                                           ld, ld, d, bias_n=st.p(self._pn(e, i, "self_attn.out_proj.bias")), resid=resid, ldr=d,
                                           drop_p=pr(c.res_dropout), drop_site=site(e.enc_id, i, S_RES1)))

    def _cross_attn_bwd(self, t, e, b, i, pr, acc1, q_src, dq_out, dq_flags):
        st, c, B, d, H, ld = self.store, self.cfg, self.B, self.cfg.d, self.cfg.H, self.ld
        Rq, Tq, Rk = b["Rl"][i], b["Tl"][i], b["Rk"]
        qpos = dict(q_pos0=0, q_stride=e.T - 1) if self._tail(b, i) else dict(q_pos0=e.q_pos0, q_stride=e.q_stride)
        GP = lambda leaf, off=0: st.gptr(self._pn(e, i, leaf), off)
        ipw = self._pn(e, i, "self_attn.in_proj_weight")
        lr = self._lowrank
        par = i & 1
        dy, dq, dao, delta = (b[n][par] for n in ("dy", "dq", "dao", "delta"))
        ldk = c.layers * ld
        dk, dv = (None, None) if lr else (b["dkall"][:, i * ld:(i + 1) * ld], b["dvall"][:, i * ld:(i + 1) * ld])
        t["c.grads"] += [dy, dq]
        t["c.acts"] += [b["ao"][i], q_src] + ([] if lr else [b["khat"], b["vhat"]])
        t["c.wg"].append(ops.gemm_problem(dy, b["ao"][i], GP("self_attn.out_proj.weight"), d, d, Rq, ld, ld, d, flags=acc1))
        t["c.dgout"].append(ops.gemm_problem(dy, st.sptr(self._pn(e, i, "self_attn.out_proj.weight")), dao, Rq, d, d, ld, ld, 0,
                                             out_kind=OUT_HEADS, heads=(B, H, Tq, self.dh, self.dhp)))
        lrx = {}
        if lr:
            HT, Sp = H * Tq, b["Sp"]
            rows = HT * B
            lrx = dict(dS=b["dSall"][i], Pd=b["Pdall"][i], xs=(Sp, Tq * B * Sp, B * Sp))
        t["c.att"].append(ops.attn_problem(b["qh"][i], b["kh"][i], b["vh"][i], b["ao"][i], ld, b["lse"][i], B, H, Tq, e.S, self.dh,
                                           self.dhp, self._mask_off(e.T_full or e.T, e.S), dO=dao, delta=delta, dQ=dq, lddq=ld,
                                           dK=dk, lddk=ldk, dV=dv, lddv=ldk, dq_scale=self.scale,
                                           drop_p=pr(e.attn_dropout), drop_site=site(e.enc_id, i, S_ATTN), **qpos, **lrx))
        t["c.wg"].append(ops.gemm_problem(dq, q_src, st.gptr(ipw, 0), d, d, Rq, ld, ld, d, flags=acc1,
                                          colsum_a=GP("self_attn.in_proj_bias")))
        if lr:
            qexp, doexp, U, Av = (b[n][par] for n in ("qexp", "doexp", "U", "Av"))
            t["c.expand"].append(ops.expand_problem(b["qh"][i], dao, qexp, doexp, B, H, Tq, self.dh, self.dhp, ld, Pd=b["Pdall"][i],
                                                    S=Sp, dbias=b["dbf"][i][d:]))
            for src, stack, dst in ((qexp, KSTACK, b["qkall"][i]), (doexp, VSTACK, b["daall"][i])):
                t["c.lrqk"].append(ops.gemm_problem(src, st.sptr(e.prefix + stack, i * ld * ld), dst, rows, d, d, ld, ld, ld,
                                                    out_kind=OUT_CT))
            for mat, hat_, dst in ((b["dSall"][i], b["khat"], U), (b["Pdall"][i], b["vhat"], Av)):
                t["c.lrqk"].append(ops.gemm_problem(mat, hat_, dst, HT, d, e.S, B * Sp, B * ld, B * ld, out_kind=OUT_CT,
                                                    flags=F_CT_NARROW, batch=(B, Sp, ld, ld)))
            t["c.wg"].append(ops.gemm_problem(qexp, U, b["dWf"][i][:d], d, d, rows, ld, ld, d))
            t["c.wg"].append(ops.gemm_problem(doexp, Av, b["dWf"][i][d:], d, d, rows, ld, ld, d))
        else:
            t["c.wg"].append(ops.gemm_problem(dk, b["khat"], b["dWf"][i][:d], d, d, Rk, ldk, ld, d, colsum_a=b["dbf"][i][:d]))
            t["c.wg"].append(ops.gemm_problem(dv, b["vhat"], b["dWf"][i][d:], d, d, Rk, ldk, ld, d, colsum_a=b["dbf"][i][d:]))
        t["c.dgq"].append(ops.gemm_problem(dq, st.sptr(ipw, 0), dq_out, Rq, d, d, ld, ld, d, flags=dq_flags))

    def _ffn_fwd(self, t, e, b, i, pr, stats):
        st, c, d, ld, ld4 = self.store, self.cfg, self.cfg.d, self.ld, self.ld4
        P = lambda leaf: st.p(self._pn(e, i, leaf))
        Rq = b["Rl"][i]
        t["f.ln"].append(ops.ln_problem(b["xmid"][i], P(f"layer_norms.{self._lnF}.weight"), P(f"layer_norms.{self._lnF}.bias"),
                                        stats[0], stats[1], Rq, out=b["xn2"][i], ldo=ld))
        t["f.fc1"].append(ops.gemm_problem(b["xn2"][i], st.sptr(self._pn(e, i, "fc1.weight")), b["h1"][i], Rq, 4 * d, d, ld, ld, ld4,
                                           bias_n=P("fc1.bias"), flags=F_RELU, drop_p=pr(c.relu_dropout),
                                           drop_site=site(e.enc_id, i, S_RELU), out_kind=OUT_CT))
        t["f.fc2"].append(ops.gemm_problem(b["h1"][i], st.sptr(self._pn(e, i, "fc2.weight")), b["x"][i + 1], Rq, d, 4 * d, ld4, ld4, d,
                                           bias_n=P("fc2.bias"), resid=b["xmid"][i], ldr=d, drop_p=pr(c.res_dropout),
                                           drop_site=site(e.enc_id, i, S_RES2)))

    def _ffn_bwd(self, t, e, b, i, pr, acc1, dx, stats):
        st, c, d, ld, ld4 = self.store, self.cfg, self.cfg.d, self.ld, self.ld4
        GP = lambda leaf: st.gptr(self._pn(e, i, leaf))
        Rq = b["Rl"][i]
        dh1, dy, dyf = b["dh1"][i & 1], b["dy"][i & 1], b["dyf"][i % 3]
        inv_relu = 1.0 / (1.0 - pr(c.relu_dropout))
        t["f.grads"] += [dyf, dh1]
        t["f.acts"] += [b["h1"][i], b["xn2"][i]]
        t["f.wg"].append(ops.gemm_problem(dyf, b["h1"][i], GP("fc2.weight"), d, 4 * d, Rq, ld, ld4, 4 * d, flags=acc1))
        t["f.dg2"].append(ops.gemm_problem(dyf, st.sptr(self._pn(e, i, "fc2.weight")), dh1, Rq, 4 * d, d, ld, ld4, ld4,
                                           gate=b["h1"][i], ldg=ld4, gate_scale=inv_relu, colsum=GP("fc1.bias"), out_kind=OUT_CT))
        t["f.wg"].append(ops.gemm_problem(dh1, b["xn2"][i], GP("fc1.weight"), 4 * d, d, Rq, ld4, ld, d, flags=acc1))
        t["f.dg1"].append(ops.gemm_problem(dh1, st.sptr(self._pn(e, i, "fc1.weight")), b["dxn"], Rq, d, 4 * d, ld4, ld, d))
        lnF = self._lnF
        t["f.ln"].append(ops.ln_problem(b["xmid"][i], st.p(self._pn(e, i, f"layer_norms.{lnF}.weight")), None, stats[0], stats[1], Rq,
                                        dy=b["dxn"], ldy=d, add=dx, dx=dx, dgamma=GP(f"layer_norms.{lnF}.weight"),
                                        dbeta=GP(f"layer_norms.{lnF}.bias"), cast=dy, ldc=ld,
                                        cast_colsum=GP("self_attn.out_proj.bias"), drop_p=pr(c.res_dropout),
                                        drop_site=site(e.enc_id, i, S_RES1)))

    def _build_fwd(self, training: bool):
        c, st, d, A = self.cfg, self.store, self.cfg.d, ops.array
        pr = (lambda p: p) if training else (lambda p: 0.0)
        ln = lambda probs: (ops.ln_fwd, self.dtype, A(LnProblem, probs), d)
        nt = lambda probs: self._gemm(GEMM_NT, probs)
        attn = lambda probs: (ops.attn_fwd, self.dtype, A(AttnProblem, probs))
        steps, kv_steps = [], []
        if self._kv_fused:
            kv_steps = [(SIDE, (ops.kv_source_fwd, self.dtype, self._kvsrc[training], self.table, d, math.sqrt(d))), (MARK, "hat")]
        elif self._kv:
            hat = []
            for b in self.buf:
                hat += [ops.ln_problem(b["ke"], self._ones, self._zeros, b["stk"][0], b["stk"][1], b["Rk"], out=b["khat"], ldo=self.ld),
                        ops.ln_problem(b["ve"], self._ones, self._zeros, b["stv"][0], b["stv"][1], b["Rk"], out=b["vhat"], ldo=self.ld)]
            kv_steps = [(SIDE, ln(hat)), (MARK, "hat")]
        for i in range(c.layers):
            t = defaultdict(list)
            for e, b in zip(self.encs, self.buf):
# ... 213 lines not shown
            t = defaultdict(list)
            for e, b in zip(self.encs, self.buf):
                dx = b["dxg"] if self._tail(b, i) else b["dx"]
                if not self._kv:
                    self._ffn_bwd(t, e, b, i, pr, ACC1, dx, (b["st1m"][i], b["st1r"][i]))
                    self._self_attn_bwd(t, e, b, i, pr, _SELF_KEYS, ACC1, ACC1)
                elif c.biprojection:
                    self._ffn_bwd(t, e, b, i, pr, ACC1, dx, (b["st2m"][i], b["st2r"][i]))
                    self._cross_attn_bwd(t, e, b, i, pr, ACC1, b["xq"][i], dx, F_ACCUM)
                    self._self_attn_bwd(t, e, b, i, pr, _BIP_SELF_KEYS, F_ACCUM, ACC1, cast=(dx, S_RES0))
                else:
                    self._ffn_bwd(t, e, b, i, pr, ACC1, dx, (b["st1m"][i], b["st1r"][i]))
                    self._cross_attn_bwd(t, e, b, i, pr, ACC1, b["xn"][i], b["dxn"], 0)
                self._ln0_bwd(t, e, b, i, pr)
            for group in (t["f.ln"], t["ln0"]):
                ops.check_ln_rows(group, d)

            def ffn(presplit, wg_late):
                w = wg(t["f.wg"], presplit)
                return [nn(t["f.dg2"])] + ([] if wg_late else [w]) + [nn(t["f.dg1"])] + ([w] if wg_late else []) + [ln(t["f.ln"])]

            def self_half(presplit):
                return [nn(t["s.dgout"]), (ops.attn_bwd, self.dtype, A(AttnProblem, t["s.att"])), wg(t["s.wg"], presplit),
                        nn(t["s.dg_a"])] + ([nn(t["s.dg_b"])] if t["s.dg_b"] else []) + ([nn(t["s.dg_c"])] if t["s.dg_c"] else []) + \
                    ([nn(t["s.dgq"]), (ops.add_n, A(AddnProblem, t["s.scatter"]))] if t["s.dgq"] else []) + [ln(t["ln0"])]

            if not self._kv:
                steps += [(WAIT, i + 2)] + ffn(t["f.acts"] if x3 else (), False) + self_half(t["s.acts"] if x3 else ()) + [(MARK, i)]
                continue
            wg_att = wg(t["c.wg"], t["c.grads"] + t["c.acts"] if x3 else ())
            dkv = (ops.attn_bwd_dkv, self.dtype, A(AttnProblem, t["c.att"]))
            steps += [(WAIT, i + 2)] + ffn(t["f.grads"] + t["f.acts"] if x3 else (), x3) + \
                [nn(t["c.dgout"]), (ops.attn_bwd_dq, self.dtype, A(AttnProblem, t["c.att"]))] + \
                ([] if lr else [(SIDE if self._dkv_side == "1" else SIDE2, dkv) if self._dkv_side in ("1", "2") else dkv]) + \
                ([] if x3 or lr else [wg_att]) + [nn(t["c.dgq"])] + ([wg_att] if x3 and not lr else [])
            if c.biprojection:
                steps += [(ops.rows_cast, self.dtype, A(CastProblem, t["s.cast"]))] + self_half(())
            else:
                steps.append(ln(t["ln0"]))
            if lr:
                steps += [(SIDE, (ops.expand_heads, self.dtype, A(ExpandProblem, t["c.expand"]))), (SIDE, nn(t["c.lrqk"])), wg_att]
            steps += [(SIDE, (ops.unfold_grads,) + self._unfold[i] + (stores and not c.biprojection,)), (MARK, i)]
        if not self._kv:
            return steps + [JOIN]
        hat, dg_kv = [], []
        for e, b in zip(self.encs, self.buf):
            if lr:
                KK, Sp = c.layers * c.H * e.T, b["Sp"]
                for mat, prod, G_ in ((b["dSall"], b["qkall"], b["Gk"]), (b["Pdall"], b["daall"], b["Gv"])):
                    dg_kv.append(ops.gemm_problem(mat, prod, G_, e.S, d, KK, self.B * Sp, self.B * self.ld, self.B * d,
                                                  batch=(self.B, Sp, self.ld, d)))
            else:
                for all_, stack, G_ in ((b["dkall"], KSTACK, b["Gk"]), (b["dvall"], VSTACK, b["Gv"])):
                    dg_kv.append(ops.gemm_problem(all_, st.sptr(e.prefix + stack), G_, b["Rk"], d, c.layers * self.ld, c.layers * self.ld,
                                                  self.ld, d))
            if not self._kv_fused:
                hat += [ops.ln_problem(b["ke"], self._ones, None, b["stk"][0], b["stk"][1], b["Rk"], dy=b["Gk"], ldy=d, dx=b["dke"]),
                        ops.ln_problem(b["ve"], self._ones, None, b["stv"][0], b["stv"][1], b["Rk"], dy=b["Gv"], ldy=d, dx=b["dve"])]
        last = (ops.kv_source_bwd, self._kvsrc[training], self.table, d, math.sqrt(d)) if self._kv_fused else ln(hat)
        return steps + [(SIDE, self._gemm(GEMM_TN if lr else GEMM_NN, dg_kv)), (SIDE, last), JOIN]

    @staticmethod
    def store_written(prefix: str, layers: int):
        return [f"{prefix}layers.{i}.{leaf}" for i in range(layers)
                for leaf in ("self_attn.in_proj_weight", "self_attn.out_proj.weight", "fc1.weight", "fc2.weight")]

    def backward(self, douts: Sequence[Optional[torch.Tensor]], on_layer=None, stores: bool = False):
        seed, training = self._last
        c, st, B, d = self.cfg, self.store, self.B, self.cfg.d
        fin, keep = [], []
        top = c.layers - 1
        self._acc0.zero_()
        for e, b, g in zip(self.encs, self.buf, douts):
            dx_top = b["dxg"] if b["tailp"] else b["dx"]
            if g is None:
                dx_top.zero_()
                b["dyf"][top % 3].zero_()
                continue
            if tuple(g.shape) != (b["Tl"][-1], B, d) or g.dtype != torch.float32:
                raise ValueError(f"encoder {e.prefix}: output gradient must be fp32 [{b['Tl'][-1]},{B},{d}], got {tuple(g.shape)} {g.dtype}")
            g = g.contiguous()
            keep.append(g)
            fin.append(ops.ln_problem(b["x"][c.layers], st.p(e.prefix + "layer_norm.weight"), None, b["stf"][0], b["stf"][1], b["Rl"][-1],
                                      dy=g, ldy=d, dx=dx_top, dgamma=st.gptr(e.prefix + "layer_norm.weight"),
                                      dbeta=st.gptr(e.prefix + "layer_norm.bias"),
                                      cast=b["dyf"][top % 3], ldc=self.ld, cast_colsum=st.gptr(self._pn(e, top, "fc2.bias")),
                                      drop_p=c.res_dropout if training else 0.0, drop_site=site(e.enc_id, top, S_RES2)))
        if fin:
            ops.ln_bwd(fin, d, self.dtype, seed)
        self._run(self._bwd[(training, stores)], seed, on_layer)
        p = c.embed_dropout if training else 0.0
        emb = []
        for e, b in zip(self.encs, self.buf):
            emb.append(ops.embed_problem(b["dx"], b["dxq"], e.T, B, drop_p=p, drop_site=site(e.enc_id, 0, S_EMB_Q)))
            if self._kv and not self._kv_fused:
                emb.append(ops.embed_problem(b["dke"], b["dxk"], e.S, B, drop_p=p, drop_site=site(e.enc_id, 0, S_EMB_K)))
                emb.append(ops.embed_problem(b["dve"], b["dxv"], e.S, B, drop_p=p, drop_site=site(e.enc_id, 0, S_EMB_V)))
        ops.embed_pos_bwd(emb, d, math.sqrt(d), seed)
        return self.input_grads()

    def merge_kv_grads(self, dests: Optional[Sequence[Optional[torch.Tensor]]] = None) -> bool:
        if not self._kv_fused:
            return False
        for i, (e, b) in enumerate(zip(self.encs, self.buf)):
            dst = dests[i] if dests is not None and dests[i] is not None else b["dxk"]
            if (tuple(dst.shape) != (e.S, self.B, self.cfg.d) or dst.dtype != torch.float32 or not dst.is_contiguous()
                    or dst.data_ptr() % 16):
                raise ValueError(f"encoder {e.prefix}: merged key / value gradient must be contiguous, 16-byte aligned fp32 "
# ... 40 lines not shown
```

biprojection-multimodal-transformer_amd/models/bpmult.py:

```python
from __future__ import annotations

import os
from typing import Dict, List, Optional, Sequence, Tuple

import torch
from torch import nn

from .. import config, ops
from .._lib import (BPM_F32, F_ACCUM, GEMM_NN, GEMM_NT, GEMM_TN, AddnProblem, CastProblem, GemmProblem, GmuProblem, TailDesc,
                    TailGrads)
from ..engine import SITE_TEXT, EncoderDesc, EncoderGroupPlan, GroupCfg, ParamStore, register_encoder_shadows
from ..graphs import _RETIRED_GRAPHS, GraphCache
from ..ops import pad32
from .encoder import TransformerEncoder

LEVEL1 = {"trans_v_with_a": ("v", "a", "a"), "trans_a_with_v": ("a", "v", "v"), "trans_v_with_l": ("v", "l", "l"),
          "trans_l_with_v": ("l", "v", "v"), "trans_a_with_l": ("a", "l", "l"), "trans_l_with_a": ("l", "a", "a")}
LEVEL2 = {"trans_l_with_v2a": ("l", "trans_a_with_v", "a"), "trans_l_with_a2v": ("l", "trans_v_with_a", "v"),
          "trans_a_with_v2l": ("a", "trans_l_with_v", "l"), "trans_a_with_l2v": ("a", "trans_v_with_l", "v"),
          "trans_v_with_a2l": ("v", "trans_l_with_a", "l"), "trans_v_with_l2a": ("v", "trans_a_with_l", "a")}
FUSE = {"l": ("trans_l_with_a2v", "trans_v_with_a", "trans_l_with_v2a", "trans_a_with_v"),
        "a": ("trans_a_with_v2l", "trans_l_with_v", "trans_a_with_l2v", "trans_v_with_l"),
        "v": ("trans_v_with_a2l", "trans_l_with_a", "trans_v_with_l2a", "trans_a_with_l")}
TIME_MAP = {"l": {"trans_v_with_a": "transfm_v2l", "trans_a_with_v": "transfm_a2l"},
# ... 194 lines not shown
            self.ones_bd = torch.ones(1, ldbd, device=dev, dtype=ct)
            self.ones_bd[:, BD:] = 0
        self.g: Dict[Tuple[str, str], dict] = {}
        for tgt in ("l", "a", "v"):
            R = self.Ng[tgt] * B
            for kind in ("mid", "top"):
                self.g[(tgt, kind)] = dict(R=R, x1=z(R, d), x2=z(R, d), xc=z(R, 2 * self.ld, dt=ct), a1=z(R, d), a2=z(R, d),
                                           ag=z(R, d), out=z(self.Ng[tgt], B, d), da1=z(R, self.ld, dt=ct),
                                           da2=z(R, self.ld, dt=ct), dag=z(R, self.ld, dt=ct), dx1=z(R, d), dx2=z(R, d))
        self._build_gmu()
        self._build_time()
        self._build_sums()
        self._conv_cache = {}
        self._conv: Dict[str, dict] = {}
        self._px_rows: Dict[str, int] = {k: 0 for k in self.N}
        n = 4 if model.four_modal else 3
        Cn = model.out_layer.out_features
        self.tail = dict(n=n, C=Cn, **{k: z(B, n * d) for k in ("x", "z", "t", "dzp", "dtp", "dx")},
                         **{k: z(B, d) for k in ("h", "p1", "y", "dy", "dp1", "dh")}, logits=z(B, Cn),
                         dextra=z(B, d) if n == 4 else None)
        self._tail_desc: Optional[TailDesc] = None
        GraphCache.__init__(self, dev)
        self.stamp = 0

    def conv_forward(self, feats: Dict[str, torch.Tensor], seed: int, training: bool) -> None:
        m, B, d, st = self.m, self.B, self.d, self.st
        packs_ct, packs_f32, gemms = [], [], []
        self._conv = {}
        for k in ("l", "a", "v"):
            x = feats[k]
            T, od = x.shape[1], x.shape[2]
            if T > self.N[k]:
                raise ValueError(f"modality {k}: sequence length {T} exceeds num_vectors_{k}={self.N[k]}")
            p = m.embed_dropout if (training and k == "l") else 0.0
            px = self.px[k]
            last = self.N[k] if self.capturing else self._px_rows[k]
            if T < last:
                px[T:last].zero_()
            self._px_rows[k] = T
            if od == d:
                packs_f32.append(ops.pack_problem(B, T, od, d, src=x, dst=px, drop_p=p, drop_site=SITE_TEXT))
                self._conv[k] = dict(T=T, od=od, x=x, p=p, packed=None)
                continue
            kp = pad32(od)
            key = (k, T)
            if key not in self._conv_cache:
                self._conv_cache[key] = dict(packed=torch.zeros(T * B, kp, device=st.device, dtype=ops.ct_torch(self.dtype)),
                                             dy=torch.zeros(T * B, self.ld, device=st.device, dtype=ops.ct_torch(self.dtype)),
                                             dpk=torch.zeros(T * B, od, device=st.device))
            cc = self._conv_cache[key]
            packs_ct.append(ops.pack_problem(B, T, od, kp, src=x, dst=cc["packed"], drop_p=p, drop_site=SITE_TEXT))
            gemms.append(ops.gemm_problem(cc["packed"], st.sptr(f"proj_{k}.weight"), px, T * B, d, od, kp, kp, d))
            self._conv[k] = dict(T=T, od=od, x=x, p=p, **cc)
        if packs_f32:
            ops.pack_rows_fwd(BPM_F32, packs_f32, seed)
        if packs_ct:
            ops.pack_rows_fwd(self.dtype, packs_ct, seed)
            ops.gemm_grouped(self.dtype, GEMM_NT, gemms, seed, x3=self.x3)

    def conv_backward(self, seed: int, need_dx: Dict[str, bool]) -> Dict[str, Optional[torch.Tensor]]:
        B, d, st = self.B, self.d, self.st
        casts, wg, dg, unpack = [], [], [], []
        res: Dict[str, Optional[torch.Tensor]] = {"l": None, "a": None, "v": None}
        for k, c in self._conv.items():
            T, od = c["T"], c["od"]
            R = T * B
            if c["packed"] is None:
                if need_dx[k]:
                    res[k] = torch.empty_like(c["x"])
                    unpack.append(ops.pack_problem(B, T, od, 0, g=self.dpx[k], ldg=d, dsrc=res[k], drop_p=c["p"], drop_site=SITE_TEXT))
                continue
            kp = pad32(od)
            casts.append(ops.cast_problem(self.dpx[k], d, R, d, dst_ct=c["dy"], ldd=self.ld))
            wg.append(ops.gemm_problem(c["dy"], c["packed"], st.gptr(f"proj_{k}.weight"), d, od, R, self.ld, kp, od,
                                       flags=F_ACCUM))
            if need_dx[k]:
                res[k] = torch.empty_like(c["x"])
                dg.append(ops.gemm_problem(c["dy"], st.sptr(f"proj_{k}.weight"), c["dpk"], R, od, d, self.ld, kp, od))
                unpack.append(ops.pack_problem(B, T, od, 0, g=c["dpk"], ldg=od, dsrc=res[k], drop_p=c["p"], drop_site=SITE_TEXT))
        if casts:
            ops.rows_cast(self.dtype, casts, seed)
            ops.gemm_grouped(self.dtype, GEMM_TN, wg, seed, x3=self.x3)
        if dg:
            ops.gemm_grouped(self.dtype, GEMM_NN, dg, seed, x3=self.x3)
        if unpack:
            ops.pack_rows_bwd(unpack, seed)
        return res

    def _build_time(self) -> None:
        B, d, st = self.B, self.d, self.st
        BD = B * d
        A = ops.array
        casts, gemms, bw_casts, bw_wg, bw_dg = [], [], [], [], []
        for (tgt, src), t in self.tmap.items():
            Ts, Td, ldbd = t["Ts"], t["Td"], t["ldbd"]
            ldw = pad32(Ts)
            W, bias = t["lin"] + ".weight", t["lin"] + ".bias"
            casts.append(ops.cast_problem(self.out1[src], BD, Ts, BD, dst_ct=t["h_ct"], ldd=ldbd))
            bw_casts.append(ops.cast_problem(t["dout"], BD, t["dout"].shape[0], BD, dst_ct=t["dout_ct"], ldd=ldbd))
            if self.prune:
                for j, r in enumerate((0, Td - 1)):
                    gemms.append(ops.gemm_problem(st.sptr(W, r * ldw), t["h_ct"], t["out"][j], 1, BD, Ts, ldw, ldbd, BD,
                                                  bias_m=st.p(bias).data_ptr() + 4 * r))
                    bw_wg.append(ops.gemm_problem(t["dout_ct"][j], t["h_ct"], st.gptr(W, r * Ts), 1, Ts, BD, ldbd, ldbd, Ts, flags=F_ACCUM))
                    bw_wg.append(ops.gemm_problem(t["dout_ct"][j], self.ones_bd, st.gptr(bias, r), 1, 1, BD, ldbd, ldbd, 1, flags=F_ACCUM))
                bw_dg.append(ops.gemm_problem(st.sptr(W), t["dout_ct"], t["dh"], Ts, BD, 2, (Td - 1) * ldw, ldbd, BD))
            else:
                gemms.append(ops.gemm_problem(st.sptr(W), t["h_ct"], t["out"], Td, BD, Ts, ldw, ldbd, BD, bias_m=st.p(bias)))
                bw_wg.append(ops.gemm_problem(t["dout_ct"], t["h_ct"], st.gptr(W), Td, Ts, BD, ldbd, ldbd, Ts, flags=F_ACCUM))
                bw_wg.append(ops.gemm_problem(t["dout_ct"], self.ones_bd, st.gptr(bias), Td, 1, BD, ldbd, ldbd, 1, flags=F_ACCUM))
                bw_dg.append(ops.gemm_problem(st.sptr(W), t["dout_ct"], t["dh"], Ts, BD, Td, ldw, ldbd, BD))
# ... 203 lines not shown
        return launches, []

    @staticmethod
    def _add_rows2(tables) -> None:
        launches, pairs = tables
        for arr in launches:
            ops.add_n(arr)
        for dst, t in pairs:
            dst[0] += t[0]
            dst[-1] += t[1]

    def backward(self, seed: int, need_dx: Dict[str, bool], stores: Optional[bool] = None):
        st = self.st
        attach = stores is None
        if stores is None:
            stores = st.begin_backward(stores=True)
        elif stores:
            ops.zero_segments(*st._zero_table)
        self.gmu_backward()
        if self.tmap:
            ops.add_n(self._sum_tmap)
            self._time_backward()
        self._ready("fuse")
        self.plan2.backward(self._d2, self._layer_hook("level2"), stores=stores)
        ops.add_n(self._sum_d1)
        self._add_rows2(self._rows2_d1)
        self.plan1.backward(self._d1, self._layer_hook("level1"), stores=stores)
        ops.add_n(self._sum_dpx)
        self._add_rows2(self._rows2_dpx)
        res = self.conv_backward(seed, need_dx)
        self._ready("proj")
        if attach:
            st.end_backward()
        return res

    def graph_forward(self, feats: Dict[str, torch.Tensor], extra: Optional[torch.Tensor], seed: int, training: bool):
        key = (training, tuple(tuple(feats[k].shape) for k in ("l", "v", "a")), extra is not None)

        def run(static, handle):
            self.forward(static, handle, training)
            return self.tail_forward(static["extra"], handle, training)

        ent = self.replay(True, key, seed, {k: feats[k] for k in ("l", "v", "a")} | {"extra": extra}, run,
                              f"BPMulT: graph capture of the forward pass failed for input shapes {key[1]} (%s); "
                              "this shape runs as eager launches",
                              on_fail=lambda: self._px_rows.update(self.N))
        if ent is None:
            return None
        if "state" not in ent:
            ent["state"] = (self._conv, self._tail_desc, self.plan1._last, self.plan2._last)
        self.plan1.maps_ready()
        self.plan2.maps_ready()
        self._px_rows = {k: feats[k].shape[1] for k in ("l", "v", "a")}
        return ent["out"][0], ent["out"][1], key

    def graph_backward(self, fkey, dlogits: torch.Tensor, dz: Optional[torch.Tensor], params, seed: int, need: Dict[str, bool]):
        self._conv, self._tail_desc, self.plan1._last, self.plan2._last = self._fg[fkey]["state"]
        fresh = self.st._fresh()
        key = (fkey, fresh, dz is not None, tuple(sorted(k for k, v in need.items() if v)))

        def run(static, handle):
            pg, dextra = self.tail_backward(static["dlogits"], static["dz"], params)
            return pg, dextra, self.backward(handle, need, stores=fresh)

        ent = self.replay(False, key, seed, {"dlogits": dlogits, "dz": dz}, run,
                              "BPMulT: graph capture of the backward pass failed (%s); this key runs as eager launches")
        if ent is None:
            return None
        self.st.end_backward()
        pg, dextra, res = ent["out"]
        return [t.clone() for t in pg], dextra, {k: (v.clone() if v is not None else None) for k, v in res.items()}

    def _ready(self, section: str, events=None) -> None:
        hook = getattr(self.m, "_grad_ready_hook", None)
        if hook is not None:
            lo, hi = self.st.sections[section]
            if hi > lo:
                hook(self.st.gflat, lo, hi, events)

    def _layer_hook(self, tag: str):
        if getattr(self.m, "_grad_ready_hook", None) is None:
            return None
        top = self.m.layers - 1

        def on_layer(i: int, events) -> None:
            if i == top:
                self._ready(f"{tag}.final", events)
            self._ready(f"{tag}.layer{i}", events)
        return on_layer


class _ModelFn(torch.autograd.Function):

    @staticmethod
    def forward(ctx, anchor, x_l, x_v, x_a, extra, model, *tail_params):
        trunk = model._trunk_for(x_l.shape[0])
        seed = model._next_seed()
        feats = {"l": x_l.detach().contiguous(), "v": x_v.detach().contiguous(), "a": x_a.detach().contiguous()}
        ex = extra.detach().contiguous() if extra is not None else None
        trunk.st.refresh_shadows()
        ran = trunk.graph_forward(feats, ex, seed, model.training) if model._graphs_on() else None
        if ran is None:
            trunk.forward(feats, seed, model.training)
            logits, z = trunk.tail_forward(ex, seed, model.training)
            ctx.fkey = None
        else:
# ... 264 lines not shown
```

biprojection-multimodal-transformer_amd/ops.py:

```python
from __future__ import annotations

import ctypes as C
import os
from typing import Optional, Sequence

import torch

from . import _lib
from ._lib import (BPM_BF16, BPM_BF16X3, BPM_F32, F_ACCUM, F_ATOMIC, F_KPAD, F_RELU, GEMM_NN, GEMM_NT, GEMM_TN, GEMM_MAX_GROUP, MAX_GROUP, OUT_CT,
                   OUT_F32, OUT_HEADS, AttnMapProblem, AttnProblem, CastProblem, EmbedProblem, GemmProblem, GmuProblem,
                   KvSourceProblem, LnProblem, PackProblem)


def pad32(n: int) -> int:
    return (n + 31) // 32 * 32


def ct_torch(dtype: int) -> torch.dtype:
    return torch.bfloat16 if dtype == BPM_BF16 else torch.float32


def _stream() -> int:
    return torch.cuda.current_stream().cuda_stream

# ... 32 lines not shown

def _counter(t, what):
    if t is not None and not isinstance(t, int) and (t.dtype != torch.int32 or t.numel() < 1):
        raise ValueError(f"{what}: an int32 device counter")
    return _p(t)


def _f32_table(t, what: str, d: int):
    if t.dtype != torch.float32 or t.dim() != 2 or t.shape[1] != d or t.stride() != (d, 1):
        raise ValueError(f"{what}: expected float32 [rows, {d}] with contiguous rows, got {t.dtype} {tuple(t.shape)}")
    return _p(t)


def _adam_scalars(what: str, ngroups: int, scale_dev, norm_dev, steps_dev, skipped_dev):
    for t, nm in ((scale_dev, "scale_dev"), (norm_dev, "norm_dev")):
        if t is not None and (t.dtype != torch.float32 or t.numel() < 1):
            raise ValueError(f"{what}: {nm}: expected float32 (one device value), got {t.dtype}")
    if steps_dev is not None and (steps_dev.dtype != torch.int32 or steps_dev.numel() < ngroups or not steps_dev.is_contiguous()):
        raise ValueError(f"{what}: steps_dev: a contiguous tensor of one int32 device counter per group")
    return _p(scale_dev), _p(norm_dev), _p(steps_dev), _counter(skipped_dev, f"{what}: skipped_dev")


def array(cls, probs: Sequence):
    return (cls * len(probs))(*probs)


def _as_array(cls, probs):
    return probs if isinstance(probs, C.Array) else array(cls, probs)


def _at(arr, i: int):
    return C.cast(C.byref(arr, i * C.sizeof(arr._type_)), C.POINTER(arr._type_))


_PROBLEM = {}


def _grouped(name: str, probs, pre=(), post=(), limit: int = MAX_GROUP, beside=None, n: Optional[int] = None) -> None:
    cls = _PROBLEM.get(name)
    if cls is None:
        cls = _PROBLEM[name] = next(t._type_ for t in _lib.SIGNATURES[name] if isinstance(t, type) and issubclass(t, C._Pointer))
    arr = _as_array(cls, probs)
    entry, s = getattr(_lib.lib(), name), _stream()
    n = len(arr) if n is None else n
    for i in range(0, n, limit):
        k = min(limit, n - i)
        also = () if beside is None else (_at(beside, i),)
        _lib.check(entry(*pre, _at(arr, i), *also, k, *(post(k) if callable(post) else post), s), name)


def gemm_problem(A, B, Cc, M: int, N: int, K: int, lda: int, ldb: int, ldc: int, *, bias_n=None, bias_m=None,
                 resid=None, ldr: int = 0, gate=None, ldg: int = 0, gate_scale: float = 1.0, alpha: float = 1.0,
                 drop_p: float = 0.0, drop_site: int = 0, colsum=None, flags: int = 0, out_kind: int = OUT_F32,
                 splitk: int = 1, heads=None, colsum_a=None, batch=None) -> GemmProblem:
    p = GemmProblem()
    p.A, p.B, p.C = (x if isinstance(x, int) else _p(x) for x in (A, B, Cc))
    p.M, p.N, p.K = M, N, K
    p.lda, p.ldb, p.ldc = lda, ldb, ldc
    p.bias_n, p.bias_m = _f32(bias_n, "bias_n"), _f32(bias_m, "bias_m")
    p.resid, p.ldr = _f32(resid, "resid"), ldr
    p.gate, p.ldg, p.gate_scale = _p(gate), ldg, gate_scale
    p.alpha, p.drop_p, p.drop_site = alpha, drop_p, drop_site
    p.colsum = colsum if isinstance(colsum, int) else _f32(colsum, "colsum")
    p.flags, p.out_kind, p.splitk = flags, out_kind, splitk
    if heads is not None:
        p.heads_B, p.heads_H, p.heads_T, p.heads_dh, p.heads_dhp = heads
    p.colsum_a = colsum_a if isinstance(colsum_a, int) else _f32(colsum_a, "colsum_a")
    if batch is not None:
        p.batch, p.batch_stride_a, p.batch_stride_b, p.batch_stride_c = batch
        p.flags |= _lib.F_BATCHED
    return p


def gemm_grouped(dtype: int, variant: int, probs, seed: int = 0, n: Optional[int] = None, x3: "Optional[X3Cache]" = None) -> None:
    arr = _as_array(GemmProblem, probs)
    cache = x3 or getattr(arr, "x3", None) or None
    if cache is not None and not isinstance(cache, X3Cache):
        raise TypeError(f"x3: an ops.X3Cache (the owner of the split images) or None, got {type(cache).__name__}")
    if cache is not None and dtype == BPM_F32 and variant in _X3_VARIANTS:
        plan = getattr(arr, "_x3_plan", None)
        if plan is None or plan.n != n or plan.cache is not cache:
            plan = _X3Plan(arr, variant, n, cache)
            arr._x3_plan = plan
        if plan.ok:
            plan.run(_lib.lib(), variant, _seed(seed), _stream())
            if plan.rest is None:
                return
            arr, n = plan.rest, None
    _grouped("bpm_gemm_grouped", arr, (dtype, variant), (_seed(seed),), GEMM_MAX_GROUP, n=n)


_X3_VARIANTS = {{"nt": GEMM_NT, "nn": GEMM_NN, "tn": GEMM_TN}[v] for v in os.environ.get("BPMULT_X3_ONLY", "nt,nn,tn").split(",") if v}


def _split(probs) -> None:
    _grouped("bpm_split_rows", probs)


class X3Cache:

    def __init__(self, device, weights: "Optional[X3Cache]" = None):
        self.device = device
        self.weights = weights
        self.images = {}
        self.static = set()
        self.static_splits = {}
        self.epoch = 0
        self.fresh = {}

    def add_static(self, lo: int, hi: int) -> None:
        self.static.add((lo, hi))

    def refresh_static(self) -> None:
        if self.static_splits:
            _split(list(self.static_splits.values()))

    def new_step(self) -> None:
        self.epoch += 1


class _X3Plan:

    def __init__(self, arr, variant: int, n: Optional[int], cache: X3Cache):
# ... 321 lines not shown
def grad_sumsq(table_dev: torch.Tensor, nseg: int, total_blocks: int, ws: torch.Tensor, out: torch.Tensor, grad_scale: float = 1.0,
               max_norm: float = 0.0, extra_sumsq: Optional[torch.Tensor] = None) -> None:
    if out.dtype != torch.float32 or out.numel() < 2 or not out.is_contiguous():
        raise ValueError("grad_sumsq: out is a contiguous float32 tensor of two elements")
    if extra_sumsq is not None and (extra_sumsq.dtype != torch.float32 or extra_sumsq.numel() != 1):
        raise ValueError("grad_sumsq: extra_sumsq is one float32 device value")
    _lib.check(_lib.lib().bpm_grad_sumsq(table_dev.data_ptr(), nseg, total_blocks, grad_scale, max_norm, _p(extra_sumsq), _p(ws),
                                         ws.numel() * ws.element_size(), _p(out), _stream()), "bpm_grad_sumsq")


def fold_bias(table_dev: torch.Tensor, ndesc: int, total_blocks: int) -> None:
    _lib.check(_lib.lib().bpm_fold_bias(table_dev.data_ptr(), ndesc, total_blocks, _stream()), "bpm_fold_bias")


def unfold_grads(table_dev: torch.Tensor, ndesc: int, total_blocks: int, store_dw: bool = False) -> None:
    _lib.check(_lib.lib().bpm_unfold_grads(table_dev.data_ptr(), ndesc, total_blocks, int(store_dw), _stream()), "bpm_unfold_grads")


def zero_table(segments):
    descs, blk = [], 0
    for ptr, n in segments:
        z = _lib.ZeroDesc()
        z.p, z.n, z.blk0 = ptr, n, blk
        blk += _blocks("bpm_zero_segment_blocks", n)
        descs.append(z)
    return device_table(descs), len(descs), blk


def zero_segments(table_dev: torch.Tensor, ndesc: int, total_blocks: int) -> None:
    _lib.check(_lib.lib().bpm_zero_segments(table_dev.data_ptr(), ndesc, total_blocks, _stream()), "bpm_zero_segments")


def embed_problem(x, out, T, B, *, accumulate=False, drop_p=0.0, drop_site=0, pos0=0, pos_stride=1) -> EmbedProblem:
    p = EmbedProblem()
    p.x, p.out, p.T, p.B = _f32(x, "embed.x"), _f32(out, "embed.out"), T, B
    p.accumulate, p.drop_p, p.drop_site = int(accumulate), drop_p, drop_site
    p.pos0, p.pos_stride = pos0, pos_stride
    return p


def embed_pos_fwd(probs, table, d, scale, seed=0) -> None:
    _grouped("bpm_embed_pos_fwd", probs, (), (_f32_table(table, "embed_pos_fwd: table", d), table.shape[0], d, scale, _seed(seed)))


def embed_pos_bwd(probs, d, scale, seed=0) -> None:
    _grouped("bpm_embed_pos_bwd", probs, (), (d, scale, _seed(seed)))


def kv_source_ok(d: int, T: int, B: int) -> bool:
    return d % 4 == 0 and 4 <= d <= 1024 and T * B * d < 1 << 32


def kv_source_problem(xk, xv, T, B, *, khat=None, vhat=None, ld=0, stats_k=(None, None), stats_v=(None, None), gk=None, gv=None,
                      dxk=None, dxv=None, drop_p=0.0, drop_site_k=0, drop_site_v=0, pos0=0, pos_stride=1) -> KvSourceProblem:
    p = KvSourceProblem()
    p.xk, p.xv, p.T, p.B, p.pos0, p.pos_stride = _f32(xk, "kv_source.xk"), _f32(xv, "kv_source.xv"), T, B, pos0, pos_stride
    p.drop_p_k, p.drop_site_k, p.drop_p_v, p.drop_site_v = drop_p, drop_site_k, drop_p, drop_site_v
    p.khat, p.vhat, p.ld = _p(khat), _p(vhat), ld
    p.mean_k, p.rstd_k = _f32(stats_k[0], "kv_source.mean_k"), _f32(stats_k[1], "kv_source.rstd_k")
    p.mean_v, p.rstd_v = _f32(stats_v[0], "kv_source.mean_v"), _f32(stats_v[1], "kv_source.rstd_v")
    p.gk, p.gv = _f32(gk, "kv_source.gk"), _f32(gv, "kv_source.gv")
    p.dxk, p.dxv = _f32(dxk, "kv_source.dxk"), _f32(dxv, "kv_source.dxv")
    return p


def set_kv_source(p: KvSourceProblem, xk, xv) -> None:
    p.xk, p.xv = _f32(xk, "kv_source.xk"), _f32(xv, "kv_source.xv")


def kv_source_fwd(dtype, probs, table, d, scale, seed=0, eps=1e-5) -> None:
    _grouped("bpm_kv_source_fwd", probs, (dtype,), (_f32_table(table, "kv_source: table", d), table.shape[0], d, scale, eps, _seed(seed)))


def kv_source_bwd(probs, table, d, scale, seed=0) -> None:
    _grouped("bpm_kv_source_bwd", probs, (), (_f32_table(table, "kv_source: table", d), table.shape[0], d, scale, _seed(seed)))


def ln_problem(x, gamma, beta, mean, rstd, R, *, out=None, ldo=0, out_f32=False, dy=None, ldy=0, add=None, dx=None,
               dgamma=None, dbeta=None, cast=None, ldc=0, cast_colsum=None, drop_p=0.0, drop_site=0) -> LnProblem:
    p = LnProblem()
    p.x, p.gamma, p.beta = _f32(x, "ln.x"), _f32(gamma, "ln.gamma"), _f32(beta, "ln.beta")
    p.out, p.ldo, p.out_f32 = _p(out), ldo, int(out_f32)
    p.mean, p.rstd, p.R = _f32(mean, "ln.mean"), _f32(rstd, "ln.rstd"), R
    p.dy, p.ldy, p.add, p.dx = _f32(dy, "ln.dy"), ldy, _f32(add, "ln.add"), _f32(dx, "ln.dx")
    p.dgamma, p.dbeta = _f32(dgamma, "ln.dgamma"), _f32(dbeta, "ln.dbeta")
    p.cast, p.ldc = _p(cast), ldc
    p.cast_colsum = cast_colsum if isinstance(cast_colsum, int) else _f32(cast_colsum, "ln.cast_colsum")
    p.drop_p, p.drop_site = drop_p, drop_site
    return p


def ln_fwd(dtype, probs, d, eps=1e-5) -> None:
    _grouped("bpm_ln_fwd", probs, (dtype,), (d, eps))


def check_ln_rows(probs, d: int) -> None:
    rows = []
    for i, p in enumerate(probs):
        for nm in ("dgamma", "dbeta", "cast_colsum"):
            a = getattr(p, nm)
            if a and (nm != "cast_colsum" or p.cast):
                rows.append((int(a), i, nm))
    rows.sort()
    for (a, i, n1), (b, j, n2) in zip(rows, rows[1:]):
        if b < a + 4 * d:
            raise ValueError(f"ln_bwd group: {n1} of problem {i} and {n2} of problem {j} share gradient words "
                             f"(0x{a:x}, 0x{b:x}; rows are {4 * d} bytes): one launch must own each row exactly once")


_LN_WS = {}


def _ln_workspace(n: int, d: int, device) -> torch.Tensor:
    key = (str(device), _stream())
    need = _lib.lib().bpm_ln_bwd_ws_bytes(n, d)
# ... 264 lines not shown
```

include/bpmult_hip.h:

```cpp
#ifndef BPMULT_HIP_H
#define BPMULT_HIP_H

#include <stddef.h>
#include <stdint.h>

#ifdef __cplusplus
extern "C" {
#endif

#define BPM_ABI_VERSION 5
#define BPM_SEED_INDIRECT (1ull << 63)
#define BPM_MAX_GROUP 18
#define BPM_GEMM_MAX_GROUP 24

enum { BPM_F32 = 0, BPM_BF16 = 1,
       BPM_BF16X3 = 2  };
enum { BPM_ERR_ARG = -1, BPM_ERR_ALIGN = -2 };

int bpm_version(void);
const char* bpm_error_string(int code);

enum { BPM_GEMM_NT = 0, BPM_GEMM_NN = 1, BPM_GEMM_TN = 2 };
enum { BPM_OUT_F32 = 0, BPM_OUT_CT = 1, BPM_OUT_HEADS = 2 };
enum { BPM_GEMM_ACCUM = 1, BPM_GEMM_RELU = 2, BPM_GEMM_ATOMIC = 4, BPM_GEMM_KPAD_ZERO = 8, BPM_GEMM_BACKGROUND = 16,
       BPM_GEMM_A_OVERLAP = 32, BPM_GEMM_B_OVERLAP = 64, BPM_GEMM_CT_NARROW = 128, BPM_GEMM_BATCHED = 256 };

typedef struct bpm_gemm_problem {
    const void* A;
    const void* B;
    void* C;
    int M, N, K;
    int lda, ldb, ldc;
    const float* bias_n;
    const float* bias_m;
    const float* resid;
    int ldr;
    const void* gate;
    int ldg;
    float gate_scale;
    float alpha;
    float drop_p;
    uint32_t drop_site;
    float* colsum;
    int flags;
    int out_kind;
    int splitk;
    int heads_B, heads_H, heads_T, heads_dh, heads_dhp;
    float* colsum_a;
    int batch, batch_stride_a, batch_stride_b, batch_stride_c;
} bpm_gemm_problem;

int bpm_gemm_grouped(int dtype, int variant, const bpm_gemm_problem* probs , int nprob,
                     uint64_t seed, void* stream);

typedef struct bpm_attn_problem {
    const void* Q; const void* K; const void* V;
    void* O; int ldo;
    float* lse;
    const void* dO;
    float* delta;
    void* dQ; int lddq;
    void* dK; int lddk;
    void* dV; int lddv;
    int B, H, T, S, dh, dhp;
    int mask_off;
    float dq_scale;
    float drop_p;
    uint32_t drop_site;
    int q_pos0, q_stride;
    void* dS; void* Pd;
    int xs_b, xs_h, xs_q;
} bpm_attn_problem;

int bpm_attn_fwd(int dtype, const bpm_attn_problem* probs , int nprob, uint64_t seed, void* stream);
int bpm_attn_bwd(int dtype, const bpm_attn_problem* probs , int nprob, uint64_t seed, void* stream);
int bpm_attn_bwd_dq(int dtype, const bpm_attn_problem* probs , int nprob, uint64_t seed, void* stream);
int bpm_attn_bwd_dkv(int dtype, const bpm_attn_problem* probs , int nprob, uint64_t seed, void* stream);

typedef struct bpm_attn_kmask {
    const uint8_t* mask;
    int ldm;
} bpm_attn_kmask;
int bpm_attn_fwd_kmask(int dtype, const bpm_attn_problem* probs , const bpm_attn_kmask* masks , int nprob,
                       uint64_t seed, void* stream);
int bpm_attn_bwd_dq_kmask(int dtype, const bpm_attn_problem* probs , const bpm_attn_kmask* masks , int nprob,
                          uint64_t seed, void* stream);
int bpm_attn_bwd_dkv_kmask(int dtype, const bpm_attn_problem* probs , const bpm_attn_kmask* masks , int nprob,
                           uint64_t seed, void* stream);

typedef struct bpm_attn_map_problem {
    const void* Q; const void* K;
    const float* lse;
    float* W; int ldw;
    int B, H, T, S, dh, dhp;
    int mask_off;
    int q_pos0, q_stride;
} bpm_attn_map_problem;

int bpm_attn_maps(int dtype, const bpm_attn_map_problem* probs , int nprob, void* stream);

typedef struct bpm_attn_amask {
    const float* mask;  int ldm;
// ... 43 lines not shown
typedef struct bpm_pack_desc {
    const void* src;
    void* dst;
    int rows, cols, ld, src_ld, dst_ld;
    unsigned blk0;
    const float* colscale;
} bpm_pack_desc;
int bpm_pack_weights(int dtype, const bpm_pack_desc* table_dev, int ndesc, unsigned total_blocks, void* stream);

typedef struct bpm_fold_desc {
    const float* W; const float* beta; const float* b; float* out;
    int rows, cols, ldw;
    unsigned blk0;
} bpm_fold_desc;
int bpm_fold_bias(const bpm_fold_desc* table_dev, int ndesc, unsigned total_blocks, void* stream);

typedef struct bpm_unfold_desc {
    const float* dWf; const float* dbf; const float* W; const float* gamma; const float* beta;
    float* dW; float* dbias; float* dgamma; float* dbeta;
    int rows, cols, ldw;
    unsigned blk0;
} bpm_unfold_desc;
int bpm_unfold_grads(const bpm_unfold_desc* table_dev, int ndesc, unsigned total_blocks, int store_dw, void* stream);

typedef struct bpm_zero_desc {
    float* p;
    unsigned n;
    unsigned blk0;
} bpm_zero_desc;
int bpm_zero_segment_blocks(unsigned n);
int bpm_zero_segments(const bpm_zero_desc* table_dev, int ndesc, unsigned total_blocks, void* stream);

typedef struct bpm_embed_problem {
    const float* x; float* out;
    int T, B;
    int accumulate;
    float drop_p; uint32_t drop_site;
    int pos0, pos_stride;
} bpm_embed_problem;
int bpm_embed_pos_fwd(const bpm_embed_problem* probs, int n, const float* table, int table_rows, int d,
                      float scale, uint64_t seed, void* stream);
int bpm_embed_pos_bwd(const bpm_embed_problem* probs, int n, int d, float scale, uint64_t seed, void* stream);

typedef struct bpm_kv_source_problem {
    const float* xk; const float* xv;
    int T, B;
    int pos0, pos_stride;
    float drop_p_k; uint32_t drop_site_k;
    float drop_p_v; uint32_t drop_site_v;
    void* khat; void* vhat; int ld;
    float* mean_k; float* rstd_k; float* mean_v; float* rstd_v;
    const float* gk; const float* gv;
    float* dxk; float* dxv;
} bpm_kv_source_problem;
int bpm_kv_source_fwd(int dtype, const bpm_kv_source_problem* probs, int n, const float* table, int table_rows, int d,
                      float scale, float eps, uint64_t seed, void* stream);
int bpm_kv_source_bwd(const bpm_kv_source_problem* probs, int n, const float* table, int table_rows, int d, float scale,
                      uint64_t seed, void* stream);

typedef struct bpm_ln_problem {
    const float* x; const float* gamma; const float* beta;
    void* out; int ldo; int out_f32;
    float* mean; float* rstd;
    int R;
    const float* dy; int ldy; const float* add; float* dx; float* dgamma; float* dbeta;
    void* cast; int ldc; float* cast_colsum; float drop_p; uint32_t drop_site;
} bpm_ln_problem;
int bpm_ln_fwd(int dtype, const bpm_ln_problem* probs, int n, int d, float eps, void* stream);
int bpm_ln_bwd(int dtype, const bpm_ln_problem* probs, int n, int d, uint64_t seed, void* stream);
size_t bpm_ln_bwd_ws_bytes(int n, int d);
int bpm_ln_bwd_ws(int dtype, const bpm_ln_problem* probs, int n, int d, uint64_t seed, void* ws, size_t ws_bytes, void* stream);

typedef struct bpm_cast_problem {
    const void* a; int lda; int a_is_ct;
    const float* b; int ldb;
    void* dst_ct; int ldd;
    int ct_cols;
    float* dst_f32; int ldf;
    float* colsum;
    int R, C;
    float drop_p; uint32_t drop_site;
} bpm_cast_problem;
int bpm_rows_cast(int dtype, const bpm_cast_problem* probs, int n, uint64_t seed, void* stream);

typedef struct bpm_gelu_problem {
    const void* u; int ldu; int u_is_ct;
    void* g; int ldg;
    const float* dg; int lddg;
    void* du; int lddu;
    int R, C;
} bpm_gelu_problem;
int bpm_gelu_fwd(int dtype, const bpm_gelu_problem* probs, int n, void* stream);
int bpm_gelu_bwd(int dtype, const bpm_gelu_problem* probs, int n, void* stream);

typedef struct bpm_bert_embed_problem {
    const int64_t* ids; const int64_t* seg;
    const float* word; const float* pos; const float* type;
    int V, P, Tt;
    const float* gamma; const float* beta;
    int B, L;
    float* x;
    void* xc; int ldc;
    float* s; float* mean; float* rstd;
    unsigned* bad;
    float drop_p; uint32_t drop_site;
} bpm_bert_embed_problem;
// ... 196 lines not shown
```

Before: 446.0 samples/s.

## Skip dead padded key/value source rows in KV projection GEMMs and layernorm

Adds live-row and live-K counts to GEMM and KV-source problems so tiles covering padded time steps beyond each modality's real length return early or skip the K loop. The KV-source LayerNorm forward writes zeros and default stats for dead rows, and its backward writes zero gradients for them. The counts are set from actual feature lengths each step. This targets work spent on padded source rows (e.g. sequences padded to 512), at the cost of extra per-tile branches and ABI struct changes that must stay consistent with the packed Prob layout.

```diff
diff --git a/biprojection-multimodal-transformer_amd/_lib.py b/biprojection-multimodal-transformer_amd/_lib.py
--- a/biprojection-multimodal-transformer_amd/_lib.py
+++ b/biprojection-multimodal-transformer_amd/_lib.py
@@ -102,7 +102,8 @@
                 ("flags", C.c_int), ("out_kind", C.c_int), ("splitk", C.c_int),
                 ("heads_B", C.c_int), ("heads_H", C.c_int), ("heads_T", C.c_int),
                 ("heads_dh", C.c_int), ("heads_dhp", C.c_int), ("colsum_a", C.c_void_p),
-                ("batch", C.c_int), ("batch_stride_a", C.c_int), ("batch_stride_b", C.c_int), ("batch_stride_c", C.c_int)]
+                ("batch", C.c_int), ("batch_stride_a", C.c_int), ("batch_stride_b", C.c_int), ("batch_stride_c", C.c_int),
+                ("a_rows_live", C.c_int), ("c_rows_live", C.c_int), ("k_live", C.c_int)]
 
 
 class AttnProblem(C.Structure):
@@ -243,7 +244,7 @@
                 ("drop_p_k", C.c_float), ("drop_site_k", C.c_uint32), ("drop_p_v", C.c_float), ("drop_site_v", C.c_uint32),
                 ("khat", C.c_void_p), ("vhat", C.c_void_p), ("ld", C.c_int),
                 ("mean_k", C.c_void_p), ("rstd_k", C.c_void_p), ("mean_v", C.c_void_p), ("rstd_v", C.c_void_p),
-                ("gk", C.c_void_p), ("gv", C.c_void_p), ("dxk", C.c_void_p), ("dxv", C.c_void_p)]
+                ("gk", C.c_void_p), ("gv", C.c_void_p), ("dxk", C.c_void_p), ("dxv", C.c_void_p), ("rows_live", C.c_int)]
 
 
 class LnProblem(C.Structure):
@@ -414,6 +415,7 @@
     L.bpm_debug_gemm_force.argtypes = [C.c_int]
     L.bpm_debug_attn_pair.argtypes = [C.c_int]
     L.bpm_debug_gemm_choice.argtypes = [C.c_int, C.c_int, C.POINTER(GemmProblem), C.c_int, C.c_int, C.POINTER(C.c_int)]
+    L.bpm_debug_gemm_work.argtypes = [C.c_int, C.c_int, C.POINTER(GemmProblem), C.c_int, C.c_int, C.POINTER(C.c_double)]
     L.bpm_debug_rows_dry.argtypes = [C.c_int]
     L.bpm_debug_rows_last.argtypes = [C.c_int, C.c_char_p, C.c_int, C.POINTER(C.c_uint), C.POINTER(C.c_uint), C.POINTER(C.c_void_p)]
     return L
diff --git a/biprojection-multimodal-transformer_amd/csrc/gemm.hip b/biprojection-multimodal-transformer_amd/csrc/gemm.hip
--- a/biprojection-multimodal-transformer_amd/csrc/gemm.hip
+++ b/biprojection-multimodal-transformer_amd/csrc/gemm.hip
@@ -1,3 +1,4 @@
+#include <algorithm>
 #include <cstdlib>
 #include <type_traits>
 
@@ -25,11 +26,16 @@
     int ldr, ldg; float gate_scale;
     float alpha;
     float* colsum;
-    float* colsum_x;
+    union {
+        float* colsum_x;
+        struct { int a_live, c_live; };
+    };
     DropCfg drop;
     int flags;
     int out_kind;
-    int hB, hH, hT, hdh, hdhp;
+    int hB, hH, hT;
+    int16_t hdh, hdhp;
+    int k_live;
     int tile0, tiles_m, tiles_n, splitk;
 };
 static_assert(sizeof(Prob) == 168, "Prob layout");
@@ -441,7 +447,14 @@
     const int nkt_all = (P.K + BK - 1) / BK;
     const int per = batched ? nkt_all : (nkt_all + P.splitk - 1) / P.splitk;
     const int kt_lo = batched ? 0 : split * per;
-    const int kt_hi = min(nkt_all, kt_lo + per);
+    int kt_hi = min(nkt_all, kt_lo + per);
+    if constexpr (XK) {
+        if (P.c_live > 0 && m0 >= P.c_live) return;
+        if (P.a_live > 0 && m0 >= P.a_live) kt_hi = kt_lo;
+    } else if constexpr (!YK) {
+        if (P.k_live > 0 && !(P.colsum_x != nullptr && n0 == 0)) kt_hi = min(kt_hi, (P.k_live + BK - 1) / BK);
+    }
+    const bool run_k = kt_lo < kt_hi || !XK;
 
     f32x4 acc[TN][TMT];
 #pragma unroll
@@ -512,7 +525,8 @@
             my_ = SY::load(Yp, ldy, n0, Nb, kt * BK, Kb, ry_, tid);
         }
     };
-    if constexpr (DEEP) {
+    if (!run_k) {
+    } else if constexpr (DEEP) {
         u32x4 rx0[SX::PER_THREAD], ry0[SY::PER_THREAD], rx1[SX::PER_THREAD], ry1[SY::PER_THREAD];
         uint32_t mx0 = 0, my0 = 0, mx1 = 0, my1 = 0;
         auto ld0 = [&](int kt) { LD(kt, rx0, ry0, mx0, my0); };
@@ -783,6 +797,13 @@
         if (q.colsum_a && (variant != BPM_GEMM_TN || q.splitk > 1)) return BPM_ERR_ARG;
         if (q.out_kind == BPM_OUT_HEADS && (q.heads_B < 1 || q.heads_dh < 1 || q.heads_H * q.heads_dh != q.N)) return BPM_ERR_ARG;
         if (q.splitk > 1 && !((q.flags & BPM_GEMM_ATOMIC) && q.out_kind == BPM_OUT_F32)) return BPM_ERR_ARG;
+        if (q.out_kind == BPM_OUT_HEADS && (q.heads_dh > 32767 || q.heads_dhp < 0 || q.heads_dhp > 32767)) return BPM_ERR_ARG;
+        if (q.a_rows_live < 0 || q.a_rows_live > q.M || q.c_rows_live < 0 || q.c_rows_live > q.M || q.k_live < 0 || q.k_live > q.K)
+            return BPM_ERR_ARG;
+        if (q.a_rows_live || q.c_rows_live || q.k_live) {
+            if (q.splitk > 1 || (q.flags & BPM_GEMM_BATCHED) || dtype == BPM_BF16X3) return BPM_ERR_ARG;
+            if (variant == BPM_GEMM_TN ? (q.a_rows_live || q.c_rows_live) : q.k_live != 0) return BPM_ERR_ARG;
+        }
         if (q.flags & BPM_GEMM_BATCHED) {
             const uintptr_t al = (uintptr_t)q.C | (uintptr_t)q.bias_n;
             if (dtype == BPM_BF16X3 || q.batch < 1 || q.batch > 4096 || q.splitk > 1 || q.out_kind == BPM_OUT_HEADS || q.bias_m || q.resid ||
@@ -882,11 +903,12 @@
         const int ntiles = (q.N + c.bn - 1) / c.bn;
         if (q.out_kind == BPM_OUT_CT && !(q.flags & BPM_GEMM_CT_NARROW) && ntiles * c.bn < q.ldc) return BPM_ERR_ARG;
         if ((q.flags & BPM_GEMM_BATCHED) && (is_dma(c.kernel) || c.kernel == K_SKINNY)) return BPM_ERR_ARG;
+        if ((q.a_rows_live || q.c_rows_live) && c.kernel == K_SKINNY) return BPM_ERR_ARG;
     }
     return 0;
 }
 
-void fill_group(const Choice& c, const bpm_gemm_problem* probs, int nprob, uint64_t seed, Group& g) {
+void fill_group(const Choice& c, int variant, const bpm_gemm_problem* probs, int nprob, uint64_t seed, Group& g) {
     g.seedp = bpm_seed_ptr(seed);
     g.nprob = nprob;
     int tile = 0;
@@ -902,9 +924,11 @@
         p.alpha = q.alpha;
         p.drop = bpm_make_drop(q.drop_p, seed, q.drop_site);
         p.colsum = q.colsum;
-        p.colsum_x = q.colsum_a;
+        p.k_live = 0;
+        if (variant == BPM_GEMM_TN) { p.colsum_x = q.colsum_a; p.k_live = q.k_live; }
+        else { p.a_live = q.a_rows_live; p.c_live = q.c_rows_live; }
         p.flags = q.flags; p.out_kind = q.out_kind;
-        p.hB = q.heads_B; p.hH = q.heads_H; p.hT = q.heads_T; p.hdh = q.heads_dh; p.hdhp = q.heads_dhp;
+        p.hB = q.heads_B; p.hH = q.heads_H; p.hT = q.heads_T; p.hdh = (int16_t)q.heads_dh; p.hdhp = (int16_t)q.heads_dhp;
         p.tile0 = tile;
         p.tiles_m = (q.M + c.bm - 1) / c.bm;
         p.tiles_n = (q.N + c.bn - 1) / c.bn;
@@ -923,15 +947,30 @@
     shape = summarise(dtype, variant, probs, nprob);
     c = choose(shape, dtype, variant, nprob, ncu ? ncu : num_cus(), g_lab);
     if (const int err = check_choice(c, probs, nprob)) return err;
-    fill_group(c, probs, nprob, seed, g);
+    fill_group(c, variant, probs, nprob, seed, g);
     return 0;
 }
 
-void work_estimate(int dtype, const bpm_gemm_problem* probs, int nprob, double& flops, double& bytes) {
+void work_estimate(int dtype, int variant, const Choice& c, const bpm_gemm_problem* probs, int nprob, double& flops, double& bytes) {
     const int sz = dtype == BPM_F32 ? 4 : 2;
+    const int kstage = c.kernel == K_DMA_TWO ? 32 : is_dma(c.kernel) ? DK : (64 / sz) * (variant == BPM_GEMM_NT ? KS_FWD : c.kernel == K_TN_LONG && BPM_DEEP_TN != 2 ? KS_WGRAD : 1);
+    auto up = [](long v, long to) { return (v + to - 1) / to * to; };
     flops = bytes = 0;
     for (int i = 0; i < nprob; ++i) {
         const bpm_gemm_problem& q = probs[i];
+        if (q.a_rows_live || q.c_rows_live || q.k_live) {
+            const double mc = q.c_rows_live ? (double)std::min<long>(q.M, up(q.c_rows_live, c.bm)) : q.M;
+            const double ma = q.a_rows_live ? std::min<double>(mc, (double)std::min<long>(q.M, up(q.a_rows_live, c.bm))) : mc;
+            const double kl = q.k_live ? (double)std::min<long>(q.K, up(q.k_live, kstage)) : q.K;
+            const double n0 = q.k_live && q.colsum_a ? std::min<double>(q.N, c.bn) : 0;
+            flops += 2.0 * ma * (n0 * q.K + (q.N - n0) * kl);
+            const double mn = mc * q.N;
+            bytes += (ma + q.N) * (n0 ? q.K : kl) * sz + mn * (q.out_kind == BPM_OUT_F32 ? 4 : sz);
+            if (q.resid) bytes += mn * 4;
+            if (q.gate) bytes += mn * sz;
+            if (q.out_kind == BPM_OUT_F32 && (q.flags & BPM_GEMM_ACCUM)) bytes += mn * 4;
+            continue;
+        }
         flops += 2.0 * q.M * (double)q.N * q.K * ((q.flags & BPM_GEMM_BATCHED) ? q.batch : 1);
         const double mn = (double)q.M * q.N;
         bytes += ((double)q.M + q.N) * q.K * sz + mn * (q.out_kind == BPM_OUT_F32 ? 4 : sz);
@@ -1013,6 +1052,16 @@
     }
     return 0;
 }
+
+extern "C" int bpm_debug_gemm_work(int dtype, int variant, const bpm_gemm_problem* probs, int nprob, int ncu, double* out) {
+    GroupShape shape;
+    Choice c;
+    Group g;
+    if (ncu < 1 || !out) return BPM_ERR_ARG;
+    if (const int err = plan_group(dtype, variant, probs, nprob, 0, ncu, shape, c, g)) return err;
+    work_estimate(dtype, variant, c, probs, nprob, out[0], out[1]);
+    return 0;
+}
 #endif
 
 #ifdef BPM_GEMM_TRACE
@@ -1028,7 +1077,7 @@
     Group g;
     if (const int err = plan_group(dtype, variant, probs, nprob, seed, 0, shape, c, g)) return err;
     double flops, bytes;
-    work_estimate(dtype, probs, nprob, flops, bytes);
+    work_estimate(dtype, variant, c, probs, nprob, flops, bytes);
     hipStream_t s = (hipStream_t)stream;
     BpmProfScope prof((is_dma(c.kernel) ? BPM_K_GEMM_DMA_NT : BPM_K_GEMM_NT) + variant, s, flops, bytes);
     return dtype == BPM_F32 ? launch<float>(c, variant, shape.xs_any, g, s) : launch<bf16_t>(c, variant, shape.xs_any, g, s);
diff --git a/biprojection-multimodal-transformer_amd/csrc/gemm_dma.h b/biprojection-multimodal-transformer_amd/csrc/gemm_dma.h
--- a/biprojection-multimodal-transformer_amd/csrc/gemm_dma.h
+++ b/biprojection-multimodal-transformer_amd/csrc/gemm_dma.h
@@ -216,10 +216,17 @@
     if (BPM_BASE_PRIO && XK && !(P.flags & BPM_GEMM_BACKGROUND)) __builtin_amdgcn_s_setprio(BPM_BASE_PRIO);
     const int m0 = (bid / P.tiles_n) * BMD, n0 = (bid % P.tiles_n) * BND;
     const int nk1 = (P.K + DKT - 1) / DKT;
-    const int nkt = X3 ? 3 * nk1 : nk1;
-
-    const __amdgpu_buffer_rsrc_t rsx = __builtin_amdgcn_make_buffer_rsrc((void*)P.X, 0, X3 ? (XK ? P.M : P.K) * P.ldx * 2 : desc_bytes(XK ? P.M : P.K, P.ldx, XK ? nkt * DKT : (P.M + 7) & ~7, 2, (P.flags & BPM_GEMM_A_OVERLAP) != 0), 0x00020000);
-    const __amdgpu_buffer_rsrc_t rsy = __builtin_amdgcn_make_buffer_rsrc((void*)P.Y, 0, X3 ? (YK ? P.N : P.K) * P.ldy * 2 : desc_bytes(YK ? P.N : P.K, P.ldy, YK ? nkt * DKT : (P.N + 7) & ~7, 2, (P.flags & BPM_GEMM_B_OVERLAP) != 0), 0x00020000);
+    const int nkt_all = X3 ? 3 * nk1 : nk1;
+    int nkt = nkt_all;
+    if constexpr (XK && !X3) {
+        if (P.c_live > 0 && m0 >= P.c_live) return;
+        if (P.a_live > 0 && m0 >= P.a_live) nkt = 0;
+    } else if constexpr (!XK && !YK && !X3) {
+        if (P.k_live > 0 && !(P.colsum_x != nullptr && n0 == 0)) nkt = min(nkt, (P.k_live + DKT - 1) / DKT);
+    }
+
+    const __amdgpu_buffer_rsrc_t rsx = __builtin_amdgcn_make_buffer_rsrc((void*)P.X, 0, X3 ? (XK ? P.M : P.K) * P.ldx * 2 : desc_bytes(XK ? P.M : P.K, P.ldx, XK ? nkt_all * DKT : (P.M + 7) & ~7, 2, (P.flags & BPM_GEMM_A_OVERLAP) != 0), 0x00020000);
+    const __amdgpu_buffer_rsrc_t rsy = __builtin_amdgcn_make_buffer_rsrc((void*)P.Y, 0, X3 ? (YK ? P.N : P.K) * P.ldy * 2 : desc_bytes(YK ? P.N : P.K, P.ldy, YK ? nkt_all * DKT : (P.N + 7) & ~7, 2, (P.flags & BPM_GEMM_B_OVERLAP) != 0), 0x00020000);
     const int vx = SX::voffset(P.ldx, m0, wave, lane), vy = SY::voffset(P.ldy, n0, wave, lane);
     const int stepx = SX::stage_step(P.ldx), stepy = SY::stage_step(P.ldy);
     const int ldx = P.ldx, ldy = P.ldy;
diff --git a/biprojection-multimodal-transformer_amd/csrc/rows_norm.hip b/biprojection-multimodal-transformer_amd/csrc/rows_norm.hip
--- a/biprojection-multimodal-transformer_amd/csrc/rows_norm.hip
+++ b/biprojection-multimodal-transformer_amd/csrc/rows_norm.hip
@@ -557,7 +557,9 @@
 namespace {
 struct KvP {
     const float* xk; const float* xv; int T, B, pos0, pstride; DropCfg dk, dv;
-    void* khat; void* vhat; int ld; float* mk; float* rk; float* mv; float* rv;
+    void* khat; void* vhat; int ld;
+    int live;
+    float* mk; float* rk; float* mv; float* rv;
     const float* gk; const float* gv; float* dxk; float* dxv;
 };
 
@@ -623,6 +625,18 @@
     const bool same = P.xk == P.xv;
     const float inv_d = 1.f / d;
     for (int row = bid * wpb + (threadIdx.x >> 6); row < R; row += nblk * wpb) {
+        if (row >= P.live) {
+            if (lane == 0) { const float rs0 = rsqrtf(eps); P.mk[row] = 0.f; P.rk[row] = rs0; P.mv[row] = 0.f; P.rv[row] = rs0; }
+#pragma unroll
+            for (int e = 0; e < NV; ++e) {
+                const int q = lane + 64 * e;
+                if (4 * q < P.ld) {
+                    put4<CT>(P.khat, (size_t)row * P.ld + 4 * q, f32x4{0.f, 0.f, 0.f, 0.f});
+                    put4<CT>(P.vhat, (size_t)row * P.ld + 4 * q, f32x4{0.f, 0.f, 0.f, 0.f});
+                }
+            }
+            continue;
+        }
         const int t = row / P.B;
         const uint32_t r0 = (uint32_t)row * (uint32_t)d;
         const float* xkr = P.xk + r0;
@@ -662,13 +676,30 @@
     const int nch = d >> 2, R = P.T * P.B;
     const bool merge = P.dxv == nullptr || P.dxv == P.dxk;
     const float inv_d = 1.f / d;
+    const int Rl = min(R, P.live);
     for (int row0 = (bid * wpb + wv) * U; row0 < R; row0 += nblk * wpb * U) {
+        if (row0 >= P.live) {
+#pragma unroll
+            for (int u = 0; u < U; ++u) {
+                if (row0 + u >= R) continue;
+                const uint32_t r0 = (uint32_t)(row0 + u) * (uint32_t)d;
+#pragma unroll
+                for (int e = 0; e < NV; ++e) {
+                    const int q = lane + 64 * e;
+                    if (q < nch) {
+                        *(f32x4*)(P.dxk + r0 + 4 * q) = f32x4{0.f, 0.f, 0.f, 0.f};
+                        if (!merge) *(f32x4*)(P.dxv + r0 + 4 * q) = f32x4{0.f, 0.f, 0.f, 0.f};
+                    }
+                }
+            }
+            continue;
+        }
         f32x4 xs[U][NS][NV], tb[U][NS][NV], g[U][2][NV];
         float mu[U][2], rs[U][2];
 #pragma unroll
         for (int u = 0; u < U; ++u) {
             const int row = row0 + u;
-            const int rc = row < R ? row : row0;
+            const int rc = row < Rl ? row : row0;
             const int t = rc / P.B;
             const uint32_t r0 = (uint32_t)rc * (uint32_t)d;
             mu[u][0] = P.mk[rc]; rs[u][0] = P.rk[rc];
@@ -697,8 +728,8 @@
 #pragma unroll
         for (int u = 0; u < U; ++u) {
             const int row = row0 + u;
-            const bool rok = row < R;
-            const uint32_t r0 = (uint32_t)(rok ? row : row0) * (uint32_t)d;
+            const bool rok = row < Rl;
+            const uint32_t r0 = (uint32_t)(row < R ? row : row0) * (uint32_t)d;
 #pragma unroll
             for (int side = 0; side < 2; ++side) {
                 const int s = SAME ? 0 : side;
@@ -730,11 +761,12 @@
                     g[u][side][e] = kv_opaque(v);
                 }
             }
-            if (!rok) continue;
+            if (row >= R) continue;
 #pragma unroll
             for (int e = 0; e < NV; ++e) {
                 const int q = lane + 64 * e;
                 if (q < nch) {
+                    if (!rok) g[u][0][e] = g[u][1][e] = f32x4{0.f, 0.f, 0.f, 0.f};
                     if (merge) {
                         *(f32x4*)(P.dxk + r0 + 4 * q) = g[u][0][e] + g[u][1][e];
                     } else {
@@ -754,6 +786,7 @@
     for (int i = 0; i < n; ++i) {
         const bpm_kv_source_problem& s = q[i];
         if (!s.xk || !s.xv || s.T < 1 || s.B < 1 || s.pos0 < 0 || s.pos_stride < 0) return BPM_ERR_ARG;
+        if (s.rows_live < 0 || (long long)s.rows_live > (long long)s.T * s.B) return BPM_ERR_ARG;
         if (!s.mean_k || !s.rstd_k || !s.mean_v || !s.rstd_v) return BPM_ERR_ARG;
         const int pstride = s.pos_stride > 0 ? s.pos_stride : 1;
         if ((long long)table_rows < (long long)s.pos0 + (long long)(s.T - 1) * pstride + 2) return BPM_ERR_ARG;
@@ -772,6 +805,7 @@
         p.dk = bpm_make_drop(s.drop_p_k, seed, s.drop_site_k);
         p.dv = bpm_make_drop(s.drop_p_v, seed, s.drop_site_v);
         p.khat = s.khat; p.vhat = s.vhat; p.ld = s.ld;
+        p.live = s.rows_live > 0 ? s.rows_live : s.T * s.B;
         p.mk = s.mean_k; p.rk = s.rstd_k; p.mv = s.mean_v; p.rv = s.rstd_v;
         p.gk = s.gk; p.gv = s.gv; p.dxk = s.dxk; p.dxv = s.dxv;
     }
diff --git a/biprojection-multimodal-transformer_amd/engine.py b/biprojection-multimodal-transformer_amd/engine.py
--- a/biprojection-multimodal-transformer_amd/engine.py
+++ b/biprojection-multimodal-transformer_amd/engine.py
@@ -431,6 +431,7 @@
 _side_streams: Dict[Tuple[int, int, bool], "torch.cuda.Stream"] = {}
 _SIDE_PRIORITY_ENV = os.environ.get("BPMULT_SIDE_PRIORITY", "auto")
 _LOWRANK = os.environ.get("BPMULT_LOWRANK", "1") != "0"
+_live_rows_on = lambda: os.environ.get("BPMULT_LIVE_ROWS", "1") != "0"
 
 
 _OPEN_FORKS: Dict[int, "torch.cuda.Stream"] = {}
@@ -477,6 +478,9 @@
         self._kv_fused = (self._kv and os.environ.get("BPMULT_KV_FUSED", "1") != "0"
                           and all(ops.kv_source_ok(d, e.S, B) for e in self.encs))
         self._kv_dst: List[Optional[torch.Tensor]] = [None] * len(self.encs)
+        self._live_on = self._kv and _live_rows_on() and not store.x3
+        self._live_sites: List[tuple] = []
+        self._live_rows: List[int] = [0] * len(self.encs)
         self._kv_keep = None
         self._lnF = 2 if cfg.biprojection else 1
         dev = store.device
@@ -498,6 +502,8 @@
                                           stats_v=b["stv"], gk=b["Gk"], gv=b["Gv"], dxk=b["dxk"], dxv=b["dxv"], drop_p=p,
                                           drop_site_k=site(e.enc_id, 0, S_EMB_K), drop_site_v=site(e.enc_id, 0, S_EMB_V))
                     for e, b in zip(self.encs, self.buf)])
+                if self._live_on:
+                    self._live_sites += [(self._kvsrc[training], j, j, "rows_live") for j in range(len(self.encs))]
         lnK = 1 if cfg.biprojection else 0
         self._unfold = []
         for i in range(L if self._kv else 0):
@@ -616,9 +622,30 @@
         for p in probs:
             p.flags |= F_KPAD | (F_BACKGROUND if background else 0)
         arr = ops.array(GemmProblem, probs)
+        for j, p in enumerate(probs):
+            if self._live_on and getattr(p, "live_site", None) is not None:
+                self._live_sites.append((arr, j) + p.live_site)
         arr.x3 = self.x3
         arr.x3_presplit = frozenset(t.data_ptr() for t in presplit)
         return (ops.gemm_grouped, self.dtype, variant, arr)
+
+    def _live(self, p, e: EncoderDesc, field: str):
+        p.live_site = (self.encs.index(e), field)
+        return p
+
+    def set_live_rows(self, t_src: Sequence[Optional[int]]) -> None:
+        if len(t_src) != len(self.encs):
+            raise ValueError(f"set_live_rows: {len(self.encs)} encoders, {len(t_src)} lengths")
+        rows = []
+        for e, t in zip(self.encs, t_src):
+            if t is not None and not 0 <= t <= e.S:
+                raise ValueError(f"encoder {e.prefix}: {t} live time steps of a key / value source of {e.S}")
+            rows.append(0 if t is None or t >= e.S or t == 0 else t * self.B)
+        if not self._live_on or rows == self._live_rows:
+            return
+        self._live_rows = rows
+        for arr, j, enc, field in self._live_sites:
+            setattr(arr[j], field, rows[enc])
 
     def _tail(self, b: dict, i: int) -> bool:
         return b["tailp"] and i == self.cfg.layers - 1
@@ -718,8 +745,9 @@
         kvf = self._pn(e, i, KVF)
         t["c.q"].append(self._proj(e, i, q_src, Rq, 0, b["qh"][i], Tq))
         for w, hat, dst in ((0, b["khat"], b["kh"][i]), (1, b["vhat"], b["vh"][i])):
-            t["c.kv"].append(ops.gemm_problem(hat, st.sptr(kvf + (".v" if w else ".k")), dst, b["Rk"], d, d, ld, ld, 0,
-                                              bias_n=st.fold(kvf, w * d, d), out_kind=OUT_HEADS, heads=(B, H, e.S, self.dh, self.dhp)))
+            t["c.kv"].append(self._live(ops.gemm_problem(hat, st.sptr(kvf + (".v" if w else ".k")), dst, b["Rk"], d, d, ld, ld, 0,
+                                                         bias_n=st.fold(kvf, w * d, d), out_kind=OUT_HEADS,
+                                                         heads=(B, H, e.S, self.dh, self.dhp)), e, "a_rows_live"))
         t["c.att"].append(ops.attn_problem(b["qh"][i], b["kh"][i], b["vh"][i], b["ao"][i], ld, b["lse"][i], B, H, Tq, e.S, self.dh,
                                            self.dhp, self._mask_off(e.T_full or e.T, e.S), drop_p=pr(e.attn_dropout),
                                            drop_site=site(e.enc_id, i, S_ATTN), **qpos))
@@ -767,8 +795,10 @@
             t["c.wg"].append(ops.gemm_problem(qexp, U, b["dWf"][i][:d], d, d, rows, ld, ld, d))
             t["c.wg"].append(ops.gemm_problem(doexp, Av, b["dWf"][i][d:], d, d, rows, ld, ld, d))
         else:
-            t["c.wg"].append(ops.gemm_problem(dk, b["khat"], b["dWf"][i][:d], d, d, Rk, ldk, ld, d, colsum_a=b["dbf"][i][:d]))
-            t["c.wg"].append(ops.gemm_problem(dv, b["vhat"], b["dWf"][i][d:], d, d, Rk, ldk, ld, d, colsum_a=b["dbf"][i][d:]))
+            t["c.wg"].append(self._live(ops.gemm_problem(dk, b["khat"], b["dWf"][i][:d], d, d, Rk, ldk, ld, d, colsum_a=b["dbf"][i][:d]),
+                                        e, "k_live"))
+            t["c.wg"].append(self._live(ops.gemm_problem(dv, b["vhat"], b["dWf"][i][d:], d, d, Rk, ldk, ld, d, colsum_a=b["dbf"][i][d:]),
+                                        e, "k_live"))
         t["c.dgq"].append(ops.gemm_problem(dq, st.sptr(ipw, 0), dq_out, Rq, d, d, ld, ld, d, flags=dq_flags))
 
     def _ffn_fwd(self, t, e, b, i, pr, stats):
@@ -1088,8 +1118,9 @@
                                                   batch=(self.B, Sp, self.ld, d)))
             else:
                 for all_, stack, G_ in ((b["dkall"], KSTACK, b["Gk"]), (b["dvall"], VSTACK, b["Gv"])):
-                    dg_kv.append(ops.gemm_problem(all_, st.sptr(e.prefix + stack), G_, b["Rk"], d, c.layers * self.ld, c.layers * self.ld,
-                                                  self.ld, d))
+                    p = ops.gemm_problem(all_, st.sptr(e.prefix + stack), G_, b["Rk"], d, c.layers * self.ld, c.layers * self.ld,
+                                         self.ld, d)
+                    dg_kv.append(self._live(p, e, "c_rows_live") if self._kv_fused else p)
             if not self._kv_fused:
                 hat += [ops.ln_problem(b["ke"], self._ones, None, b["stk"][0], b["stk"][1], b["Rk"], dy=b["Gk"], ldy=d, dx=b["dke"]),
                         ops.ln_problem(b["ve"], self._ones, None, b["stv"][0], b["stv"][1], b["Rk"], dy=b["Gv"], ldy=d, dx=b["dve"])]
diff --git a/biprojection-multimodal-transformer_amd/models/bpmult.py b/biprojection-multimodal-transformer_amd/models/bpmult.py
--- a/biprojection-multimodal-transformer_amd/models/bpmult.py
+++ b/biprojection-multimodal-transformer_amd/models/bpmult.py
@@ -270,11 +270,15 @@
             packs_ct.append(ops.pack_problem(B, T, od, kp, src=x, dst=cc["packed"], drop_p=p, drop_site=SITE_TEXT))
             gemms.append(ops.gemm_problem(cc["packed"], st.sptr(f"proj_{k}.weight"), px, T * B, d, od, kp, kp, d))
             self._conv[k] = dict(T=T, od=od, x=x, p=p, **cc)
+        self._set_live_rows({k: feats[k].shape[1] for k in ("l", "a", "v")})
         if packs_f32:
             ops.pack_rows_fwd(BPM_F32, packs_f32, seed)
         if packs_ct:
             ops.pack_rows_fwd(self.dtype, packs_ct, seed)
             ops.gemm_grouped(self.dtype, GEMM_NT, gemms, seed, x3=self.x3)
+
+    def _set_live_rows(self, T: Dict[str, int]) -> None:
+        self.plan1.set_live_rows([T[kv] for (q, kv, _) in LEVEL1.values()])
 
     def conv_backward(self, seed: int, need_dx: Dict[str, bool]) -> Dict[str, Optional[torch.Tensor]]:
         B, d, st = self.B, self.d, self.st
@@ -584,6 +588,7 @@
         self.plan1.maps_ready()
         self.plan2.maps_ready()
         self._px_rows = {k: feats[k].shape[1] for k in ("l", "v", "a")}
+        self._set_live_rows(self._px_rows)
         return ent["out"][0], ent["out"][1], key
 
     def graph_backward(self, fkey, dlogits: torch.Tensor, dz: Optional[torch.Tensor], params, seed: int, need: Dict[str, bool]):
diff --git a/biprojection-multimodal-transformer_amd/ops.py b/biprojection-multimodal-transformer_amd/ops.py
--- a/biprojection-multimodal-transformer_amd/ops.py
+++ b/biprojection-multimodal-transformer_amd/ops.py
@@ -108,7 +108,8 @@
 def gemm_problem(A, B, Cc, M: int, N: int, K: int, lda: int, ldb: int, ldc: int, *, bias_n=None, bias_m=None,
                  resid=None, ldr: int = 0, gate=None, ldg: int = 0, gate_scale: float = 1.0, alpha: float = 1.0,
                  drop_p: float = 0.0, drop_site: int = 0, colsum=None, flags: int = 0, out_kind: int = OUT_F32,
-                 splitk: int = 1, heads=None, colsum_a=None, batch=None) -> GemmProblem:
+                 splitk: int = 1, heads=None, colsum_a=None, batch=None, a_rows_live: int = 0, c_rows_live: int = 0,
+                 k_live: int = 0) -> GemmProblem:
     p = GemmProblem()
     p.A, p.B, p.C = (x if isinstance(x, int) else _p(x) for x in (A, B, Cc))
     p.M, p.N, p.K = M, N, K
@@ -125,6 +126,7 @@
     if batch is not None:
         p.batch, p.batch_stride_a, p.batch_stride_b, p.batch_stride_c = batch
         p.flags |= _lib.F_BATCHED
+    p.a_rows_live, p.c_rows_live, p.k_live = a_rows_live, c_rows_live, k_live
     return p
 
 
@@ -552,7 +554,7 @@
 
 
 def kv_source_problem(xk, xv, T, B, *, khat=None, vhat=None, ld=0, stats_k=(None, None), stats_v=(None, None), gk=None, gv=None,
-                      dxk=None, dxv=None, drop_p=0.0, drop_site_k=0, drop_site_v=0, pos0=0, pos_stride=1) -> KvSourceProblem:
+                      dxk=None, dxv=None, drop_p=0.0, drop_site_k=0, drop_site_v=0, pos0=0, pos_stride=1, rows_live=0) -> KvSourceProblem:
     p = KvSourceProblem()
     p.xk, p.xv, p.T, p.B, p.pos0, p.pos_stride = _f32(xk, "kv_source.xk"), _f32(xv, "kv_source.xv"), T, B, pos0, pos_stride
     p.drop_p_k, p.drop_site_k, p.drop_p_v, p.drop_site_v = drop_p, drop_site_k, drop_p, drop_site_v
@@ -561,6 +563,7 @@
     p.mean_v, p.rstd_v = _f32(stats_v[0], "kv_source.mean_v"), _f32(stats_v[1], "kv_source.rstd_v")
     p.gk, p.gv = _f32(gk, "kv_source.gk"), _f32(gv, "kv_source.gv")
     p.dxk, p.dxv = _f32(dxk, "kv_source.dxk"), _f32(dxv, "kv_source.dxv")
+    p.rows_live = rows_live
     return p
 
 
diff --git a/include/bpmult_hip.h b/include/bpmult_hip.h
--- a/include/bpmult_hip.h
+++ b/include/bpmult_hip.h
@@ -48,6 +48,7 @@
     int heads_B, heads_H, heads_T, heads_dh, heads_dhp;
     float* colsum_a;
     int batch, batch_stride_a, batch_stride_b, batch_stride_c;
+    int a_rows_live, c_rows_live, k_live;
 } bpm_gemm_problem;
 
 int bpm_gemm_grouped(int dtype, int variant, const bpm_gemm_problem* probs , int nprob,
@@ -197,6 +198,7 @@
     float* mean_k; float* rstd_k; float* mean_v; float* rstd_v;
     const float* gk; const float* gv;
     float* dxk; float* dxv;
+    int rows_live;
 } bpm_kv_source_problem;
 int bpm_kv_source_fwd(int dtype, const bpm_kv_source_problem* probs, int n, const float* table, int table_rows, int d,
                       float scale, float eps, uint64_t seed, void* stream);
```

Result: no change. 448.1 samples/s, median of 5 (+0.5%).
